# p768lwy3/torecsys

Hardware: AMD Instinct MI355X
Metric: CTR samples/sec fwd+bwd (DeepFM, 39 fields x dim 64) (higher is better)
Workload: dtype bf16; 1 GPU; BASELINE.json configs[1]: DeepFM 39 Criteo-shaped fields, MLP [400,400,400], 1000000 total rows, embed_dim 64, batch 65536, uniform indices, uniform field sizes; global_batch=65536, rows=1000000, parallelism=single, microbatches=1, optimizer=none, hipgraph=True, hipgraph_input_sets=1, hipgraph_steps_per_replay=4, fused_lookup_fm=True

## Files before the change

include/trs_abi.h:

```cpp
#ifndef TRS_ABI_H_
#define TRS_ABI_H_

#include <stddef.h>
#include <stdint.h>

#ifdef __cplusplus
extern "C" {
#endif

#define TRS_ABI_VERSION 3

enum { TRS_F32 = 0, TRS_BF16 = 1 };
enum { TRS_I64 = 0, TRS_I32 = 1 };
enum {
  TRS_OK = 0,
  TRS_EINVAL = -1,
  TRS_EDTYPE = -2,
  TRS_ESHAPE = -3,
  TRS_EALIGN = -4,
  TRS_ELAUNCH = -5,
  TRS_EWORKSPACE = -6
};

typedef void* trs_stream_t;
// ... 160 lines not shown
int trs_cin_bwd(const void* x0, const void* xk, const void* Wc, const void* gy, int64_t B, int32_t N,
                int32_t H, int32_t C, int32_t E, int32_t dtype, float* dWc, void* dx0, void* dxk,
                int32_t accumulate_dx0, trs_stream_t stream);

size_t trs_cin_cl_workspace_bytes(int32_t N, int32_t H, int32_t C);
int trs_cin_cl_fwd(const void* x0T, int32_t ld0, const void* xkT, int32_t ldk, const void* Wc,
                   const void* bias, int64_t B, int32_t N, int32_t H, int32_t C, int32_t E, int32_t dtype,
                   int32_t tri, void* yT, void* workspace, size_t ws_bytes, trs_stream_t stream);
size_t trs_cin_cl_bwd_data_workspace_bytes(int32_t N, int32_t H, int32_t C);
int trs_cin_cl_bwd_data(const void* x0T, int32_t ld0, const void* xkT, int32_t ldk, const void* gyT,
                        const void* Wc, int64_t B, int32_t N, int32_t H, int32_t C, int32_t E,
                        int32_t dtype, int32_t tri, void* dx0T, void* dxkT, int32_t ldo, void* workspace,
                        size_t ws_bytes, trs_stream_t stream);

size_t trs_cin_dw_workspace_bytes(int64_t B, int32_t N, int32_t H, int32_t C);
int trs_cin_dw(const void* gy, const void* x0, const void* xk, int64_t B, int32_t N, int32_t H, int32_t C,
               int32_t E, int32_t dtype, int32_t tri, float* dW, void* workspace, size_t ws_bytes,
               trs_stream_t stream);

int trs_cin_cl_bwd_data_live(const void* x0T, int32_t ld0, const void* xkT, int32_t ldk, const void* gyT, int32_t ldg,
                             const void* Wc, int64_t B, int32_t N, int32_t H, int32_t C, int32_t E, int32_t dtype,
                             void* dx0T, void* dxkT, int32_t ldo, void* workspace, size_t ws_bytes, trs_stream_t stream);
int trs_cin_dw_live(const void* gy, int64_t gy_batch_stride, const void* x0, const void* xk, int64_t B, int32_t N, int32_t H,
                    int32_t C, int32_t E, int32_t dtype, float* dW, void* workspace, size_t ws_bytes, trs_stream_t stream);

size_t trs_relu_bwd_bias_workspace_bytes(int64_t rows, int32_t C);
int trs_relu_bwd_bias(const void* gy, const void* y, int64_t rows, int32_t C, int32_t dtype, void* gz,
                      float* gb, void* workspace, size_t ws_bytes, trs_stream_t stream);

int trs_mlp_fused_supported(int32_t num_layers, const int32_t* widths);
#define TRS_MLP_FAMILY_AUTO 0
#define TRS_MLP_FAMILY_TILE 1
#define TRS_MLP_FAMILY_ROW_OWNER 2
#define TRS_MLP_FAMILY_MIXED 3
int32_t trs_mlp_fused_family(int32_t num_layers, const int32_t* widths, int64_t rows, int32_t request);
size_t trs_mlp_fused_workspace_bytes(int32_t num_layers, const int32_t* widths);
size_t trs_mlp_fused_mask_bytes(int64_t rows);
int trs_mlp_fused_fwd(const void* x, int64_t rows, int32_t num_layers, const int32_t* widths,
                      const void* const* weights, const void* const* biases, void* const* hidden, void* const* masks,
                      void* mask_in, void* y, int32_t dtype, int32_t family, int32_t x_stride, void* workspace,
                      size_t ws_bytes, trs_stream_t stream);
int trs_mlp_fused_bwd_data(const void* gy, int64_t rows, int32_t num_layers, const int32_t* widths,
                           const void* const* weights, const void* const* masks, void* const* gz, float* const* gbias,
                           void* gx, const void* mask_in, float* gbias_in, int32_t dtype, int32_t family,
                           void* workspace, size_t ws_bytes, trs_stream_t stream);
size_t trs_mlp_fused_bwd_wlast_part_bytes(int32_t num_layers, const int32_t* widths, int64_t rows, int32_t dtype,
                                          int32_t family, int32_t live);
int trs_mlp_fused_bwd_data_wlast(const void* gy, int32_t gy_stride, int64_t rows, int32_t num_layers,
                                 const int32_t* widths, const void* const* weights, const void* const* masks,
                                 void* const* gz, float* const* gbias, void* gx, const void* mask_in, float* gbias_in,
                                 const void* h_last, int32_t h_stride, int32_t live, float* wl_part,
                                 size_t wl_part_bytes, float* gw_last, int32_t dtype, int32_t family, void* workspace,
                                 size_t ws_bytes, trs_stream_t stream);

int trs_pad_cols(const void* src, int32_t c_in, void* dst, int32_t c_out, int64_t rows, int32_t dtype,
                 trs_stream_t stream);

size_t trs_rows_gemm_workspace_bytes(int32_t out_f, int32_t in_f);
int trs_rows_gemm_supported(int32_t out_f, int32_t in_f, int32_t x_stride);
int trs_rows_gemm(const void* x, int64_t rows, int32_t x_stride, const void* W, int32_t out_f, int32_t in_f,
                  int32_t dtype, void* y, void* workspace, size_t ws_bytes, trs_stream_t stream);

size_t trs_bucket_workspace_bytes(int64_t BN, int32_t world);
int trs_bucket_by_owner(const void* idx, int32_t idx_dtype, const int64_t* offsets, int64_t B, int32_t N,
                        int64_t rows_per_rank, int32_t world, int64_t* counts, int32_t* send_ids,
                        int32_t* send_pos, int32_t* inv_pos, void* workspace, size_t ws_bytes,
                        trs_stream_t stream);
int trs_embed_fm_sharded(const void* back, int64_t back_rows, const void* local, int64_t local_rows, int64_t n_valid,
                         int32_t E, int32_t dtype, const int32_t* inv_pos, const int32_t* send_ids, int32_t self_lo,
                         int32_t self_n, int64_t B, int32_t N, void* emb, void* fm, float* fm_sum, int32_t* err_flag,
                         trs_stream_t stream);
int trs_permute_grad(const void* g_block, const void* g_fm, const float* fm_sum, const void* x,
                     const int32_t* pos, int64_t K, int32_t N, int32_t E, int32_t dtype, void* out,
                     trs_stream_t stream);

int trs_bag_route_count(const void* idx, int32_t idx_dtype, int64_t B, int32_t L, int64_t V, int64_t rows_per_rank,
                        int32_t world, int32_t* counts, int32_t* err_flag, trs_stream_t stream);
int trs_bag_route_place(const void* idx, int32_t idx_dtype, int64_t B, int32_t L, int64_t V, int64_t rows_per_rank,
                        int32_t world, const int32_t* seg_start, int32_t* send_ids, int64_t n_send, trs_stream_t stream);
int trs_bag_pool_segments(const void* shard, int64_t n_valid, int32_t E, int32_t dtype, const int32_t* ids, int64_t n,
                          const int32_t* seg_start, int64_t S, float* out, int32_t* err_flag, trs_stream_t stream);
int trs_bag_combine(const float* parts, int32_t P, int64_t B, int32_t E, float scale, int32_t dtype, void* out,
                    trs_stream_t stream);
int trs_bag_expand_grad(const void* g_all, int32_t dtype, int32_t E, const int32_t* ids, int64_t n,
                        const int32_t* seg_start, int64_t S, int64_t n_valid, int64_t pad_local_row, void* grad_rows,
                        int32_t* ids_bwd, trs_stream_t stream);

int trs_rowdot_fwd(const void* h, const void* w, const void* bias, int64_t rows, int32_t C, int32_t dtype, void* out,
                   trs_stream_t stream);
size_t trs_rowdot_bwd_workspace_bytes(int64_t rows, int32_t C);
int trs_rowdot_bwd(const void* g, const void* h, const void* w, int64_t rows, int32_t C, int32_t dtype, void* gh,
                   float* gw, float* gb, void* workspace, size_t ws_bytes, trs_stream_t stream);

int trs_transpose_pad(const void* in, int64_t B, int32_t R, int32_t Cc, int32_t ld_in, void* out, int32_t ld_out,
                      int32_t dtype, trs_stream_t stream);

int trs_cat_head_fwd(const void* a, const void* d, const void* w, const void* bias, int64_t rows, int32_t N, int32_t Ea,
                     int32_t Eb, int32_t dtype, void* out, trs_stream_t stream);
size_t trs_cat_head_bwd_workspace_bytes(int64_t rows, int32_t N, int32_t Ea, int32_t Eb);
int trs_cat_head_bwd(const void* g, const void* a, const void* d, const void* w, int64_t rows, int32_t N, int32_t Ea,
                     int32_t Eb, int32_t dtype, void* ga, void* gd, float* gw, float* gb, void* workspace,
                     size_t ws_bytes, trs_stream_t stream);

int trs_wgrad_finish(const float* part, int32_t S, int32_t R, int32_t Cc, int32_t out_rows, int32_t out_cols,
                     int32_t dtype, void* gw, const float* gb_f32, void* gb, trs_stream_t stream);
int trs_wgrad_finish_t(const float* part, int32_t S, int32_t Cc, int32_t R, int32_t out_rows, int32_t out_cols,
                       int32_t dtype, void* gw, const float* gb_f32, void* gb, trs_stream_t stream);
int32_t trs_wgrad_rows_splits(int32_t M, int32_t N, int64_t rows);
int trs_wgrad_rows(const void* g, int32_t ldg, const void* x, int32_t ldx, int64_t rows, int32_t M, int32_t N,
                   int32_t dtype, int32_t S, float* part, trs_stream_t stream);
int32_t trs_wgrad_rows_many_splits(int32_t n_jobs, const int32_t* M, const int32_t* N, const int32_t* ldg,
                                   const int32_t* ldx, int64_t rows);
int32_t trs_wgrad_rows_many_map(int32_t n_jobs, const int32_t* M, const int32_t* N, const int32_t* ldg,
                                const int32_t* ldx, int64_t rows, int32_t block, int64_t* out);
int trs_wgrad_rows_many(int32_t n_jobs, const void* const* g, const int32_t* ldg, const void* const* x,
                        const int32_t* ldx, int64_t rows, const int32_t* M, const int32_t* N, int32_t S,
                        float* const* part, trs_stream_t stream);
int trs_wgrad_finish_many(int32_t n_jobs, const float* const* part, int32_t S, const int32_t* R, const int32_t* Cc,
                          const int32_t* out_rows, const int32_t* out_cols, int32_t dtype, void* const* gw,
                          const float* const* gb_f32, void* const* gb, trs_stream_t stream);
int32_t trs_wgrad_wide_splits(int32_t M_x, int32_t N_g, int32_t ld_g, int64_t rows);
int trs_wgrad_wide(const void* x, int32_t ldx, const void* g, int32_t ldg, int64_t rows, int32_t M_x, int32_t N_g,
                   int32_t S, float* part, trs_stream_t stream);
int32_t trs_wgrad_wide_many_splits(int32_t n_jobs, const int32_t* M_x, const int32_t* ldx, const int32_t* N_g,
                                   const int32_t* ldg, int64_t rows);
int32_t trs_wgrad_wide_many_map(int32_t n_jobs, const int32_t* M_x, const int32_t* ldx, const int32_t* N_g,
                                const int32_t* ldg, int64_t rows, int32_t block, int64_t* out);
int trs_wgrad_wide_many(int32_t n_jobs, const void* const* x, const int32_t* ldx, const void* const* g,
                        const int32_t* ldg, int64_t rows, const int32_t* M_x, const int32_t* N_g, int32_t S,
                        float* const* part, trs_stream_t stream);
int trs_wgrad_finish_t_many(int32_t n_jobs, const float* const* part, int32_t S, const int32_t* Cc, const int32_t* R,
                            const int32_t* out_rows, const int32_t* out_cols, int32_t dtype, void* const* gw,
                            const float* const* gb_f32, void* const* gb, trs_stream_t stream);
int trs_copy_padded_many(const int64_t* desc, int32_t n, int32_t elem_size, int64_t max_elems, trs_stream_t stream);

int32_t trs_cin_glue_blocks(int64_t B);
int trs_cin_glue_stats(const void* y, int64_t B, int32_t E, int32_t C, int32_t dtype, float* partial,
                       trs_stream_t stream);
int trs_cin_glue_fwd(const void* y, const float* scale, const float* shift, int64_t B, int32_t E, int32_t C, int32_t D,
                     int32_t Hs, int32_t dtype, void* hidden, void* pooled, trs_stream_t stream);
int trs_cin_glue_bwd_reduce(const void* y, const void* g_hidden, const void* g_pooled, const float* scale,
                            const float* shift, const float* mean, const float* invstd, int64_t B, int32_t E, int32_t C,
                            int32_t D, int32_t Hs, int32_t dtype, float* partial, trs_stream_t stream);
int trs_cin_glue_bwd_apply(const void* y, const void* g_hidden, const void* g_pooled, const float* scale,
                           const float* shift, const float* mean, const float* invstd, const float* c1, const float* c2,
                           int64_t B, int32_t E, int32_t C, int32_t D, int32_t Hs, int32_t dtype, void* gy,
                           trs_stream_t stream);
int trs_cin_glue_cf_supported(int32_t E, int32_t C);
int trs_cin_glue_fwd_cf(const void* y, const float* scale, const float* shift, int64_t B, int32_t E, int32_t C,
                        int32_t D, int32_t Hs, int32_t dtype, void* hidden, void* hidden_cf, void* pooled,
                        trs_stream_t stream);
int trs_cin_glue_bwd_apply_cf(const void* y, const void* g_hidden, const void* g_pooled, const float* scale,
                              const float* shift, const float* mean, const float* invstd, const float* c1,
                              const float* c2, int64_t B, int32_t E, int32_t C, int32_t D, int32_t Hs, int32_t dtype,
                              void* gy, void* gy_cf, float* colsum_partial, trs_stream_t stream);

int trs_opn_vec_fwd(const void* x, const void* kern, int32_t kern_is_num, int64_t B, int32_t N, int32_t E,
                    int32_t dtype, void* out, trs_stream_t stream);
size_t trs_opn_vec_bwd_workspace_bytes(int64_t B, int32_t N, int32_t E);
int trs_opn_vec_bwd(const void* g, const void* x, const void* kern, int32_t kern_is_num, int64_t B, int32_t N,
                    int32_t E, int32_t dtype, void* gx, float* gkern_vec, void* workspace, size_t ws_bytes,
                    trs_stream_t stream);

int trs_pair_mul_fwd(const void* a, const void* c, const void* bias, int32_t bias_per_pair, int64_t B, int32_t N,
                     int32_t E, int32_t dtype, void* out, trs_stream_t stream);
int trs_pair_mul_bwd(const void* g, const void* a, const void* c, int64_t B, int32_t N, int32_t E, int32_t dtype,
                     void* ga, void* gc, trs_stream_t stream);

int trs_rows_mul_bias_fwd(const void* a, const void* c, const void* bias, int32_t bias_per_pair, int64_t rows,
                          int32_t P, int32_t E, int32_t dtype, void* out, trs_stream_t stream);
int trs_rows_mul_bwd(const void* g, const void* a, const void* c, int64_t rows, int32_t E, int32_t dtype, void* ga,
                     void* gc, trs_stream_t stream);

int trs_pair_bilinear_fwd(const void* x, const void* W, int32_t w_per_pair, const void* bias, int32_t bias_per_pair,
                          int32_t mode, int64_t B, int32_t N, int32_t E, int32_t dtype, void* out,
                          trs_stream_t stream);
int trs_pair_bilinear_bwd_data(const void* g, const void* x, const void* W, int32_t w_per_pair, int32_t mode,
                               int64_t B, int32_t N, int32_t E, int32_t dtype, void* gx, void* gT,
                               trs_stream_t stream);

int trs_pair_bilinear_fwd_mfma(const void* x, const void* Wt, const void* bias, const int32_t* tasks, int32_t ntasks,
                               int32_t mode, int64_t B, int32_t N, int32_t E, int32_t dtype, void* out,
                               trs_stream_t stream);

int trs_pair_bilinear_bwd_data_mfma(const void* g, const void* x, const void* W, const void* Wt,
                                    const int32_t* tasks_i, int32_t nti, const int32_t* seg_i,
// ... 132 lines not shown
```

torecsys_amd/_abi.py:

```python
from __future__ import annotations

import ctypes
import os
import threading
from ctypes import c_char_p, c_int32, c_int64, c_size_t, c_void_p

import torch

_HERE = os.path.dirname(os.path.abspath(__file__))
LIB_PATH = os.environ.get("TRS_LIB_PATH") or os.path.join(_HERE, "libtrs_hip.so")

TRS_F32, TRS_BF16 = 0, 1
TRS_I64, TRS_I32 = 0, 1

_P, _I32, _I64, _SZ, _F32 = c_void_p, c_int32, c_int64, c_size_t, ctypes.c_float

_OPTIMIZER_TAIL = [_I32, _F32, _P, _F32, _F32, _F32, _P, _P, _P, _SZ, _P]

SIGNATURES = {
    "trs_version": (c_int32, []),
    "trs_last_error_string": (c_char_p, []),
    "trs_rowdot_fwd": (c_int32, [_P, _P, _P, _I64, _I32, _I32, _P, _P]),
    "trs_rowdot_bwd_workspace_bytes": (_SZ, [_I64, _I32]),
    "trs_rowdot_bwd": (c_int32, [_P, _P, _P, _I64, _I32, _I32, _P, _P, _P, _P, _SZ, _P]),
    "trs_transpose_pad": (c_int32, [_P, _I64, _I32, _I32, _I32, _P, _I32, _I32, _P]),
    "trs_cat_head_fwd": (c_int32, [_P, _P, _P, _P, _I64, _I32, _I32, _I32, _I32, _P, _P]),
    "trs_cat_head_bwd_workspace_bytes": (_SZ, [_I64, _I32, _I32, _I32]),
    "trs_cat_head_bwd": (c_int32, [_P, _P, _P, _P, _I64, _I32, _I32, _I32, _I32, _P, _P, _P, _P, _P, _SZ, _P]),
    "trs_wgrad_finish": (c_int32, [_P, _I32, _I32, _I32, _I32, _I32, _I32, _P, _P, _P, _P]),
    "trs_wgrad_finish_t": (c_int32, [_P, _I32, _I32, _I32, _I32, _I32, _I32, _P, _P, _P, _P]),
    "trs_wgrad_rows_splits": (c_int32, [_I32, _I32, _I64]),
    "trs_wgrad_rows": (c_int32, [_P, _I32, _P, _I32, _I64, _I32, _I32, _I32, _I32, _P, _P]),
    "trs_wgrad_rows_many_splits": (c_int32, [_I32, _P, _P, _P, _P, _I64]),
    "trs_wgrad_rows_many_map": (c_int32, [_I32, _P, _P, _P, _P, _I64, _I32, _P]),
    "trs_wgrad_rows_many": (c_int32, [_I32, _P, _P, _P, _P, _I64, _P, _P, _I32, _P, _P]),
    "trs_wgrad_finish_many": (c_int32, [_I32, _P, _I32, _P, _P, _P, _P, _I32, _P, _P, _P, _P]),
    "trs_wgrad_wide_splits": (c_int32, [_I32, _I32, _I32, _I64]),
    "trs_wgrad_wide": (c_int32, [_P, _I32, _P, _I32, _I64, _I32, _I32, _I32, _P, _P]),
    "trs_wgrad_wide_many_splits": (c_int32, [_I32, _P, _P, _P, _P, _I64]),
    "trs_wgrad_wide_many_map": (c_int32, [_I32, _P, _P, _P, _P, _I64, _I32, _P]),
    "trs_wgrad_wide_many": (c_int32, [_I32, _P, _P, _P, _P, _I64, _P, _P, _I32, _P, _P]),
    "trs_wgrad_finish_t_many": (c_int32, [_I32, _P, _I32, _P, _P, _P, _P, _I32, _P, _P, _P, _P]),
    "trs_copy_padded_many":(c_int32, [_P, _I32, _I32, _I64, _P]),
    "trs_cin_glue_blocks": (c_int32, [_I64]),
    "trs_cin_glue_stats": (c_int32, [_P, _I64, _I32, _I32, _I32, _P, _P]),
    "trs_cin_glue_fwd": (c_int32, [_P, _P, _P, _I64, _I32, _I32, _I32, _I32, _I32, _P, _P, _P]),
    "trs_cin_glue_bwd_reduce": (c_int32, [_P, _P, _P, _P, _P, _P, _P, _I64, _I32, _I32, _I32, _I32, _I32, _P, _P]),
    "trs_cin_glue_bwd_apply": (c_int32, [_P, _P, _P, _P, _P, _P, _P, _P, _P, _I64, _I32, _I32, _I32, _I32, _I32, _P, _P]),
    "trs_cin_glue_cf_supported": (c_int32, [_I32, _I32]),
    "trs_cin_glue_fwd_cf": (c_int32, [_P, _P, _P, _I64, _I32, _I32, _I32, _I32, _I32, _P, _P, _P, _P]),
    "trs_cin_glue_bwd_apply_cf": (c_int32, [_P, _P, _P, _P, _P, _P, _P, _P, _P, _I64, _I32, _I32, _I32, _I32, _I32, _P, _P, _P,
                                            _P]),
    "trs_opn_vec_fwd": (c_int32, [_P, _P, _I32, _I64, _I32, _I32, _I32, _P, _P]),
    "trs_opn_vec_bwd_workspace_bytes": (_SZ, [_I64, _I32, _I32]),
    "trs_opn_vec_bwd": (c_int32, [_P, _P, _P, _I32, _I64, _I32, _I32, _I32, _P, _P, _P, _SZ, _P]),
    "trs_pair_mul_fwd": (c_int32, [_P, _P, _P, _I32, _I64, _I32, _I32, _I32, _P, _P]),
    "trs_rows_mul_bias_fwd": (c_int32, [_P, _P, _P, _I32, _I64, _I32, _I32, _I32, _P, _P]),
    "trs_rows_mul_bwd": (c_int32, [_P, _P, _P, _I64, _I32, _I32, _P, _P, _P]),
    "trs_pair_mul_bwd": (c_int32, [_P, _P, _P, _I64, _I32, _I32, _I32, _P, _P, _P]),
    "trs_pair_bilinear_fwd": (c_int32, [_P, _P, _I32, _P, _I32, _I32, _I64, _I32, _I32, _I32, _P, _P]),
    "trs_pair_bilinear_bwd_data": (c_int32, [_P, _P, _P, _I32, _I32, _I64, _I32, _I32, _I32, _P, _P, _P]),
    "trs_pair_bilinear_fwd_mfma": (c_int32, [_P, _P, _P, _P, _I32, _I32, _I64, _I32, _I32, _I32, _P, _P]),
    "trs_pair_bilinear_bwd_data_mfma": (c_int32, [_P, _P, _P, _P, _P, _I32, _P, _P, _I32, _P, _I32, _I64, _I32, _I32, _I32,
                                                  _P, _P, _P, _P]),
    "trs_pair_bilinear_bwd_w_mfma_workspace_bytes": (_SZ, [_I64, _I32, _I32]),
    "trs_pair_bilinear_bwd_w_mfma": (c_int32, [_P, _P, _I32, _I64, _I32, _I32, _I32, _P, _P, _SZ, _P]),
    "trs_pair_epilogue_fwd": (c_int32, [_P, _P, _P, _I32, _I32, _I64, _I32, _I32, _I32, _P, _P]),
    "trs_pair_epilogue_bwd": (c_int32, [_P, _P, _P, _I32, _I64, _I32, _I32, _I32, _P, _P]),
    "trs_afm_fwd_dropout": (c_int32, [_P, _P, _P, _P, _P, _P, _F32, _I64, _I32, _I32, _I32, _I32, _P, _P, _P, _P]),
    "trs_afm_bwd_dropout": (c_int32, [_P, _P, _P, _P, _P, _F32, _P, _P, _P, _I64, _I32, _I32, _I32, _I32, _P, _P, _P, _P,
                                      _P, _P, _SZ, _P]),
    "trs_afm_pair_tiles": (c_int32, [_I32, _P, _I32, _P]),
    "trs_pad_cols": (c_int32, [_P, _I32, _P, _I32, _I64, _I32, _P]),
    "trs_rows_gemm_workspace_bytes": (_SZ, [_I32, _I32]),
    "trs_rows_gemm_supported": (c_int32, [_I32, _I32, _I32]),
    "trs_rows_gemm": (c_int32, [_P, _I64, _I32, _P, _I32, _I32, _I32, _P, _P, _SZ, _P]),
    "trs_afm_bwd_workspace_bytes": (_SZ, [_I64, _I32, _I32, _I32]),
    "trs_pack_columns": (c_int32, [_P, _P, _I32, _I32, _I64, _P, _I32, _P]),
    "trs_mark_timestamp": (c_int32, [_P, _I32, _P]),
    "trs_wall_clock_khz": (_I64, []),
    "trs_gather_rows": (c_int32, [_P, _I64, _I32, _I32, _P, _I32, _P, _I64, _I32, _P, _P, _P]),
    "trs_gather_rows_tables": (c_int32, [_P, _P, _I32, _I32, _P, _I32, _I64, _I32, _P, _P, _P]),
    "trs_fa_gather_rows": (c_int32, [_P, _I64, _I32, _I32, _P, _I32, _P, _I64, _I32, _P, _P, _P]),
    "trs_csr_workspace_bytes": (_SZ, [_I64, _I64]),
    "trs_csr_build": (c_int32, [_P, _I32, _P, _I64, _I32, _I64, _P, _P, _P, _SZ, _P, _P]),
    "trs_csr_build_skip": (c_int32, [_P, _I32, _P, _I64, _I32, _I64, _I64, _P, _P, _P, _SZ, _P, _P]),
    "trs_scatter_workspace_bytes": (_SZ, [_I64, _I32, _I32, _I32]),
    "trs_scatter_rows": (c_int32, [_P, _I64, _P, _I32, _P, _P, _P, _P, _I64, _I64, _I32, _I32, _I32, _I64, _P, _P, _SZ, _P]),
    "trs_scatter_rows_first": (c_int32, [_P, _I64, _P, _I32, _P, _P, _P, _P, _I64, _I64, _I32, _I32, _I32, _I64, _P, _P, _P, _P,
                                         _SZ, _P]),
    "trs_scatter_rows_update": (c_int32, [_P, _I64, _P, _I32, _P, _P, _P, _P, _I64, _I64, _I32, _I32, _I32, _I64,
                                          *_OPTIMIZER_TAIL]),
    "trs_scatter_rows_update_mapped": (c_int32, [_P, _P, _P, _P, _P, _I64, _I64, _I64, _I32, _I32, *_OPTIMIZER_TAIL]),
    "trs_adam_step_size": (c_int32, [_P, _P, ctypes.c_double, ctypes.c_double, _P, _P]),
    "trs_compact_rows_slots": (_I64, [_I64]),
# ... 43 lines not shown
    "trs_senet_bwd_workspace_bytes": (_SZ, [_I64, _I32, _I32]),
    "trs_senet_bwd": (c_int32, [_P, _P, _P, _P, _P, _P, _I64, _I32, _I32, _I32, _I32, _P, _P, _P, _P, _P, _P, _SZ, _P]),
    "trs_senet_squeeze": (c_int32, [_P, _I64, _I32, _I32, _I32, _P, _P]),
    "trs_senet_scale_fwd": (c_int32, [_P, _P, _I64, _I32, _I32, _I32, _P, _P]),
    "trs_senet_scale_bwd": (c_int32, [_P, _P, _P, _P, _I64, _I32, _I32, _I32, _P, _P, _P]),
    "trs_moe_gate_vector_shape": (c_int32, [_I32, _I32]),
    "trs_moe_gate_last_path": (c_int32, []),
    "trs_moe_gate_fwd": (c_int32, [_P, _P, _P, _I64, _I32, _I32, _I32, _P, _P]),
    "trs_moe_gate_bwd": (c_int32, [_P, _P, _P, _P, _I64, _I32, _I32, _I32, _P, _P, _P]),
    "trs_dynamic_routing_path": (c_int32, [_I32, _I32, _I32, _I32]),
    "trs_dynamic_routing_fwd": (c_int32, [_P, _P, _I64, _I32, _I32, _I32, _I32, _I32, _P, _P, _P, _P]),
    "trs_dynamic_routing_bwd": (c_int32, [_P, _P, _P, _P, _I64, _I32, _I32, _I32, _I32, _P, _P]),
    "trs_seq_rnn_path": (c_int32, [_I32, _I32, _I32, _I32]),
    "trs_seq_rnn_workspace_bytes": (_SZ, [_I32, _I32]),
    "trs_seq_rnn_fwd": (c_int32, [_P, _I64, _I32, _I32, _P, _I32, _P, _I32, _I64, _I32, _P, _P, _P, _P, _I32, _I32, _I32, _P,
                                  _P, _P, _P, _P, _SZ, _P, _P]),
    "trs_seq_rnn_bwd": (c_int32, [_P, _I64, _I32, _I32, _P, _I32, _P, _I32, _I64, _I32, _P, _P, _P, _P, _I32, _I32, _P, _P,
                                  _P, _P, _P, _P, _P, _SZ, _P]),
    "trs_fm_fwd": (c_int32, [_P, _I64, _I32, _I32, _I32, _P, _P, _P]),
    "trs_fm_bwd": (c_int32, [_P, _P, _P, _I64, _I32, _I32, _I32, _P, _P]),
    "trs_pair_dot_fwd": (c_int32, [_P, _I64, _I32, _I32, _I32, _P, _P]),
    "trs_embed_pair_dot": (c_int32, [_P, _I64, _I32, _I32, _P, _I32, _P, _I64, _I32, _P, _P, _P, _P]),
    "trs_pair_dot_bwd": (c_int32, [_P, _P, _I64, _I32, _I32, _I32, _P, _P]),
    "trs_ffm_fwd": (c_int32, [_P, _I64, _I32, _I32, _I32, _P, _P]),
    "trs_ffm_bwd": (c_int32, [_P, _P, _I64, _I32, _I32, _I32, _P, _P]),
    "trs_ffm_fused_fwd": (c_int32, [_P, _I64, _I32, _I32, _P, _I32, _P, _I64, _I32, _P, _P, _P]),
    "trs_ffm_fused_bwd": (c_int32, [_P, _I64, _I32, _I32, _P, _I32, _P, _P, _P, _P, _I64, _I32, _P, _P, _P]),
    "trs_cross_workspace_bytes": (_SZ, [_I64, _I32, _I32, _I32]),
    "trs_cross_fwd": (c_int32, [_P, _P, _P, _I64, _I32, _I32, _I32, _P, _P, _SZ, _P]),
    "trs_cross_bwd": (c_int32, [_P, _P, _P, _P, _I64, _I32, _I32, _I32, _I32, _P, _P, _P, _P, _SZ, _P]),
    "trs_cin_fwd": (c_int32, [_P, _P, _P, _P, _I64, _I32, _I32, _I32, _I32, _I32, _P, _P, _P]),
    "trs_cin_bwd": (c_int32, [_P, _P, _P, _P, _I64, _I32, _I32, _I32, _I32, _I32, _P, _P, _P, _I32, _P]),
    "trs_cin_cl_workspace_bytes": (_SZ, [_I32, _I32, _I32]),
    "trs_cin_cl_fwd": (c_int32, [_P, _I32, _P, _I32, _P, _P, _I64, _I32, _I32, _I32, _I32, _I32, _I32, _P, _P, _SZ, _P]),
    "trs_cin_cl_bwd_data_workspace_bytes": (_SZ, [_I32, _I32, _I32]),
    "trs_cin_cl_bwd_data": (c_int32, [_P, _I32, _P, _I32, _P, _P, _I64, _I32, _I32, _I32, _I32, _I32, _I32, _P, _P, _I32,
                                      _P, _SZ, _P]),
    "trs_cin_dw_workspace_bytes": (_SZ, [_I64, _I32, _I32, _I32]),
    "trs_cin_dw": (c_int32, [_P, _P, _P, _I64, _I32, _I32, _I32, _I32, _I32, _I32, _P, _P, _SZ, _P]),
    "trs_cin_cl_bwd_data_live": (c_int32, [_P, _I32, _P, _I32, _P, _I32, _P, _I64, _I32, _I32, _I32, _I32, _I32, _P, _P, _I32,
                                           _P, _SZ, _P]),
    "trs_cin_dw_live": (c_int32, [_P, _I64, _P, _P, _I64, _I32, _I32, _I32, _I32, _I32, _P, _P, _SZ, _P]),
    "trs_relu_bwd_bias_workspace_bytes": (_SZ, [_I64, _I32]),
    "trs_relu_bwd_bias": (c_int32, [_P, _P, _I64, _I32, _I32, _P, _P, _P, _SZ, _P]),
    "trs_mlp_fused_supported": (c_int32, [_I32, _P]),
    "trs_mlp_fused_family": (c_int32, [_I32, _P, _I64, _I32]),
    "trs_mlp_fused_workspace_bytes": (_SZ, [_I32, _P]),
    "trs_mlp_fused_mask_bytes": (_SZ, [_I64]),
    "trs_mlp_fused_fwd": (c_int32, [_P, _I64, _I32, _P, _P, _P, _P, _P, _P, _P, _I32, _I32, _I32, _P, _SZ, _P]),
    "trs_mlp_fused_bwd_data": (c_int32, [_P, _I64, _I32, _P, _P, _P, _P, _P, _P, _P, _P, _I32, _I32, _P, _SZ, _P]),
    "trs_mlp_fused_bwd_wlast_part_bytes": (_SZ, [_I32, _P, _I64, _I32, _I32, _I32]),
    "trs_mlp_fused_bwd_data_wlast": (c_int32, [_P, _I32, _I64, _I32, _P, _P, _P, _P, _P, _P, _P, _P, _P, _I32, _I32, _P, _SZ, _P,
                                               _I32, _I32, _P, _SZ, _P]),
    "trs_ctr_logit_fwd": (c_int32, [_P, _I32, _P, _I32, _P, _P, _I32, _P, _I64, _I32, _P, _P]),
    "trs_bce_logits_workspace_bytes": (_SZ, [_I64]),
    "trs_bce_logits_fwd": (c_int32, [_P, _I32, _P, _I32, _I64, _P, _P, _SZ, _P]),
    "trs_bce_logits_bwd": (c_int32, [_P, _I32, _P, _I32, _P, _I64, _P, _P]),
    "trs_pair_score_path": (c_int32, [_I32, _I32]),
    "trs_embed_pair_score_fwd": (c_int32, [_P, _I64, _P, _I64, _P, _I64, _P, _I64, _I32, _I32, _I32, _I64, _I32, _I32, _P,
                                           _I32, _P, _P]),
    "trs_pair_score_bwd_workspace_bytes": (_SZ, [_I64, _I32, _I32, _I32]),
    "trs_embed_pair_score_bwd": (c_int32, [_P, _I64, _P, _I64, _P, _I64, _P, _I64, _I32, _I32, _I32, _I64, _I32, _I32, _P,
                                           _I32, _P, _P, _SZ, _P]),
    "trs_rank_loss_workspace_bytes": (_SZ, [_I64]),
    "trs_rank_loss_fwd": (c_int32, [_P, _I64, _P, _I64, _I32, _P, _I64, _I32, _I32, _F32, _I32, _P, _P, _P, _SZ, _P]),
    "trs_rank_loss_bwd": (c_int32, [_P, _I64, _P, _I64, _I32, _P, _I64, _I32, _I32, _F32, _I32, _P, _P, _P, _I64, _P, _I64,
                                    _P]),
    "trs_bucket_workspace_bytes": (_SZ, [_I64, _I32]),
    "trs_bucket_by_owner": (c_int32, [_P, _I32, _P, _I64, _I32, _I64, _I32, _P, _P, _P, _P, _P, _SZ, _P]),
    "trs_embed_fm_sharded": (c_int32, [_P, _I64, _P, _I64, _I64, _I32, _I32, _P, _P, _I32, _I32, _I64, _I32, _P, _P, _P, _P,
                                       _P]),
    "trs_permute_grad": (c_int32, [_P, _P, _P, _P, _P, _I64, _I32, _I32, _I32, _P, _P]),
    "trs_bag_route_count": (c_int32, [_P, _I32, _I64, _I32, _I64, _I64, _I32, _P, _P, _P]),
    "trs_bag_route_place": (c_int32, [_P, _I32, _I64, _I32, _I64, _I64, _I32, _P, _P, _I64, _P]),
    "trs_bag_pool_segments": (c_int32, [_P, _I64, _I32, _I32, _P, _I64, _P, _I64, _P, _P, _P]),
    "trs_bag_combine": (c_int32, [_P, _I32, _I64, _I32, _F32, _I32, _P, _P]),
    "trs_bag_expand_grad": (c_int32, [_P, _I32, _I32, _P, _I64, _P, _I64, _I64, _I64, _P, _P, _P]),
}

_lib = None
_lock = threading.Lock()


def load() -> ctypes.CDLL:
    global _lib
    if _lib is not None:
        return _lib
    with _lock:
        if _lib is not None:
            return _lib
        if not os.path.exists(LIB_PATH):
            raise RuntimeError(
                f"torecsys_amd: HIP library not built ({LIB_PATH} missing). Run "
                "`python -m torecsys_amd.build` (or __graft_entry__.build()). There is no CPU fallback.")
        lib = ctypes.CDLL(LIB_PATH)
        for name, (res, args) in SIGNATURES.items():
            try:
                fn = getattr(lib, name)
            except AttributeError as e:
                raise RuntimeError(f"torecsys_amd: {LIB_PATH} does not export {name}; rebuild it") from e
            fn.restype = res
            fn.argtypes = args
        _lib = lib
    return _lib


# ... 52 lines not shown
            _HipEvent._free.append(self.h)
            self.h = None


_MARK_CAP = 4096
_rings = {}


def _mark_ring(name: str) -> torch.Tensor:
    r = _rings.get(name)
    if r is None:
        raise RuntimeError(f"time_kernel({name!r}) must be enabled before the capture starts")
    return r


_every = {}


def time_kernel(name: str, enable: bool = True, expect: int = 0, every: int = 1):
    if enable:
        _timed[name] = []
        _every[name] = [max(1, int(every)), 0]
        _rings[name] = torch.zeros(_MARK_CAP + 1, dtype=torch.int64, device="cuda")
        fresh = [_HipEvent() for _ in range(max(0, 2 * expect - len(_HipEvent._free)))]
        for ev in fresh:
            ev.release()
    else:
        _timed.pop(name, None)
        _rings.pop(name, None)
        _every.pop(name, None)


def kernel_times_ms(name: str):
    torch.cuda.synchronize()
    ev = _timed.get(name, [])
    out = [a.elapsed_time(b) for a, b in ev]
    for a, b in ev:
        a.release()
        b.release()
    ev.clear()
    ring = _rings.get(name)
    if ring is not None:
        host = ring.cpu()
        n = int(host[0])
        if n > _MARK_CAP:
            n = 0
        khz = float(load().trs_wall_clock_khz())
        if khz > 0:
            out += [float(host[2 + 2 * j] - host[1 + 2 * j]) / khz for j in range(n // 2)]
        ring.zero_()
    return out


def call(name: str, *args):
    rec = _timed.get(name)
    if rec is not None:
        st = stream_ptr()
        if torch.cuda.is_current_stream_capturing():
            ring = _mark_ring(name)
            lib = load()
            lib.trs_mark_timestamp(ctypes.c_void_p(ring.data_ptr()), _MARK_CAP, st)
            rc = getattr(lib, name)(*args)
            lib.trs_mark_timestamp(ctypes.c_void_p(ring.data_ptr()), _MARK_CAP, st)
        else:
            ev = _every[name]
            ev[1] += 1
            if ev[1] % ev[0] == 0:
                a, b = _HipEvent(), _HipEvent()
                a.record(st, 0)
                rc = getattr(load(), name)(*args)
                b.record(st, 0)
                rec.append((a, b))
            else:
                rc = getattr(load(), name)(*args)
    else:
        rc = getattr(load(), name)(*args)
    if rc != 0:
        raise RuntimeError(f"{name} failed (code {rc}): {last_error()}")


def size_query(name: str, *args) -> int:
    return int(getattr(load(), name)(*args))


def value_dtype_code(t: torch.Tensor) -> int:
    if t.dtype == torch.float32:
        return TRS_F32
    if t.dtype == torch.bfloat16:
        return TRS_BF16
    raise TypeError(f"torecsys_amd: unsupported value dtype {t.dtype} (float32 and bfloat16 only)")


def index_dtype_code(t: torch.Tensor) -> int:
    if t.dtype == torch.int64:
        return TRS_I64
    if t.dtype == torch.int32:
        return TRS_I32
    raise TypeError(f"torecsys_amd: unsupported index dtype {t.dtype}")


def current_stream_of(dev: torch.device) -> torch.cuda.Stream:
    return torch.cuda.current_stream(dev.index if dev.index is not None else torch._C._cuda_getDevice())


def require_device(*tensors: torch.Tensor) -> torch.device:
    dev = None
    for t in tensors:
        if t is None:
            continue
        if not t.is_cuda:
            raise RuntimeError(
                "torecsys_amd: tensors must be on a HIP ('cuda') device; this package has no CPU path "
                f"(got a tensor on {t.device})")
        if dev is None:
            dev = t.device
        elif t.device != dev:
            raise RuntimeError(f"torecsys_amd: tensors on different devices ({dev} vs {t.device})")
    if dev is not None and dev.index is not None and dev.index != torch._C._cuda_getDevice():
# ... 13 lines not shown
```

torecsys_amd/csrc/mlp_epilogue.hip:

```cpp
#include <algorithm>

#include "trs_common.hpp"

namespace trs {

constexpr int RB_THREADS = 256;

template <typename T>
__global__ __launch_bounds__(RB_THREADS) void relu_bwd_bias_kernel(const uint4* __restrict__ gy, const uint4* __restrict__ y,
                                                                   uint4* __restrict__ gz, float* __restrict__ part,
                                                                   int64_t rows, int vpr ,
                                                                   int rows_per_band) {
  constexpr int VE = Vec16<T>::VE;
  __shared__ float red[RB_THREADS][VE];
  const int64_t r0 = (int64_t)blockIdx.x * rows_per_band;
  const int64_t r1 = r0 + rows_per_band < rows ? r0 + rows_per_band : rows;
  const int cv = threadIdx.x % vpr, rl = threadIdx.x / vpr, rstep = RB_THREADS / vpr;
  float acc[VE];
#pragma unroll
  for (int k = 0; k < VE; ++k) acc[k] = 0.f;
  if (rl < rstep) {
    constexpr int U = 4;
    for (int64_t rb = r0 + rl; rb < r1; rb += (int64_t)rstep * U) {
      uint4 gv[U], yv[U];
// ... 158 lines not shown
        if (v == 0) gb += gr[u];
      }
      if (gh != nullptr) {
        float o[VE];
#pragma unroll
        for (int k = 0; k < VE; ++k) o[k] = gr[u] * wv[k];
        gh[r * lpr + v] = Vec16<T>::pack(o);
      }
    }
  }
  if (partial == nullptr) return;
#pragma unroll
  for (int k = 0; k < VE; ++k) red[threadIdx.x][k] = gw[k];
  red[threadIdx.x][VE] = gb;
  __syncthreads();
  if (rr == 0) {
    float* mine = partial + (size_t)blockIdx.x * (C + 1);
#pragma unroll
    for (int k = 0; k < VE; ++k) {
      float t = 0.f;
      for (int q = 0; q < rpp; ++q) t += red[q * lpr + v][k];
      mine[v * VE + k] = t;
    }
    if (v == 0) {
      float t = 0.f;
      for (int q = 0; q < rpp; ++q) t += red[q * lpr][VE];
      mine[C] = t;
    }
  }
}

__global__ void rowdot_finish_kernel(const float* __restrict__ tmp, int C, float* __restrict__ gw,
                                         float* __restrict__ gb) {
  const int c = blockIdx.x * blockDim.x + threadIdx.x;
  if (c < C) gw[c] = tmp[c];
  else if (c == C) gb[0] = tmp[C];
}

static int rowdot_fwd_blocks(int64_t rows, int lpr) {
  const int rpp = 256 / lpr;
  return (int)std::min<int64_t>((rows + (int64_t)rpp * 4 - 1) / ((int64_t)rpp * 4), 8192);
}
static int rowdot_blocks(int64_t rows, int lpr) {
  const int rpp = 256 / lpr;
  return (int)std::min<int64_t>((rows + rpp - 1) / rpp, 1023);
}
static bool rowdot_shape_ok(int C, int dtype) {
  const int ve = dtype == TRS_F32 ? 4 : 8;
  const int lpr = C % ve == 0 ? C / ve : 0;
  return lpr >= 1 && lpr <= 64 && (lpr & (lpr - 1)) == 0;
}

template <typename T>
__device__ __forceinline__ void wgrad_finish_body(const float* __restrict__ part, int S, int R, int Cc, int out_rows,
                                                  int out_cols, T* __restrict__ gw, const float* __restrict__ gbf,
                                                  T* __restrict__ gb) {
  const int c = blockIdx.x * 256 + threadIdx.x;
  if ((int)blockIdx.y == out_rows) {
    if (gb != nullptr && c < out_rows) gb[c] = from_f32<T>(gbf[c]);
    return;
  }
  if ((int)blockIdx.y > out_rows || c >= out_cols) return;
  const int r = blockIdx.y;
  const float* p = part + (size_t)r * Cc + c;
  const size_t stride = (size_t)R * Cc;
  float a0 = 0.f, a1 = 0.f, a2 = 0.f, a3 = 0.f;
  int s = 0;
  for (; s + 4 <= S; s += 4) {
    a0 += p[(size_t)s * stride];
    a1 += p[(size_t)(s + 1) * stride];
    a2 += p[(size_t)(s + 2) * stride];
    a3 += p[(size_t)(s + 3) * stride];
  }
  for (; s < S; ++s) a0 += p[(size_t)s * stride];
  gw[(size_t)r * out_cols + c] = from_f32<T>((a0 + a1) + (a2 + a3));
}

template <typename T>
__global__ __launch_bounds__(256) void wgrad_finish_kernel(const float* __restrict__ part, int S, int R, int Cc,
                                                          int out_rows, int out_cols, T* __restrict__ gw,
                                                          const float* __restrict__ gbf, T* __restrict__ gb) {
  wgrad_finish_body<T>(part, S, R, Cc, out_rows, out_cols, gw, gbf, gb);
}

constexpr int WF_MAXJ = 8;
struct WgradFinishJob {
  const float* part;
  void* gw;
  const float* gbf;
  void* gb;
  int R, Cc, out_rows, out_cols;
};
struct WgradFinishArgs {
  WgradFinishJob job[WF_MAXJ];
  int S;
};
template <typename T>
__global__ __launch_bounds__(256) void wgrad_finish_many_kernel(WgradFinishArgs a) {
  const WgradFinishJob& j = a.job[blockIdx.z];
  if (j.part == nullptr) {
    const int c = blockIdx.x * 256 + threadIdx.x;
    if (blockIdx.y == 0 && c < j.out_cols) ((T*)j.gb)[c] = from_f32<T>(j.gbf[c]);
    return;
  }
  wgrad_finish_body<T>(j.part, a.S, j.R, j.Cc, j.out_rows, j.out_cols, (T*)j.gw, j.gbf, (T*)j.gb);
}

constexpr int WF_SL = 16;
constexpr int WF_COLS = 256 / WF_SL;
template <typename T>
__global__ __launch_bounds__(256) void wgrad_finish_few_rows_kernel(const float* __restrict__ part, int S, int R, int Cc,
                                                                   int out_rows, int out_cols, T* __restrict__ gw,
                                                                   const float* __restrict__ gbf, T* __restrict__ gb) {
  __shared__ float red[WF_SL][WF_COLS + 1];
  if ((int)blockIdx.y == out_rows) {
    const int c = blockIdx.x * 256 + threadIdx.x;
    if (gb != nullptr && c < out_rows) gb[c] = from_f32<T>(gbf[c]);
    return;
  }
  const int cl = threadIdx.x % WF_COLS, sl = threadIdx.x / WF_COLS;
  const int c = blockIdx.x * WF_COLS + cl;
  const int r = blockIdx.y;
  const size_t stride = (size_t)R * Cc;
  float a0 = 0.f, a1 = 0.f, a2 = 0.f, a3 = 0.f;
  if (c < out_cols) {
    const float* p = part + (size_t)r * Cc + c;
    int s = sl;
    for (; s + 3 * WF_SL < S; s += 4 * WF_SL) {
      a0 += p[(size_t)s * stride];
      a1 += p[(size_t)(s + WF_SL) * stride];
      a2 += p[(size_t)(s + 2 * WF_SL) * stride];
      a3 += p[(size_t)(s + 3 * WF_SL) * stride];
    }
    for (; s < S; s += WF_SL) a0 += p[(size_t)s * stride];
  }
  red[sl][cl] = (a0 + a1) + (a2 + a3);
  __syncthreads();
  if (sl == 0 && c < out_cols) {
    float t = 0.f;
#pragma unroll
    for (int k = 0; k < WF_SL; ++k) t += red[k][cl];
    gw[(size_t)r * out_cols + c] = from_f32<T>(t);
  }
}

template <typename T>
__device__ __forceinline__ void wgrad_finish_t_body(const float* __restrict__ part, int S, int Cc, int R, int out_rows,
                                                    int out_cols, T* __restrict__ gw, const float* __restrict__ gbf,
                                                    T* __restrict__ gb) {
  __shared__ float tile[32][33];
  const int tx = threadIdx.x & 31, ty = threadIdx.x >> 5;
  if ((int)blockIdx.y == (out_cols + 31) / 32) {
    const int r = blockIdx.x * 32 + tx;
    if (gb != nullptr && ty == 0 && r < out_rows) gb[r] = from_f32<T>(gbf[r]);
    return;
  }
  const int r0 = blockIdx.x * 32, c0 = blockIdx.y * 32;
  const size_t stride = (size_t)Cc * R;
  float acc[4] = {0.f, 0.f, 0.f, 0.f};
#pragma unroll
  for (int i = 0; i < 4; ++i) {
    const int c = c0 + ty + 8 * i, r = r0 + tx;
    if (c < out_cols && r < out_rows) {
      const float* p = part + (size_t)c * R + r;
      float a0 = 0.f, a1 = 0.f;
      int sidx = 0;
      for (; sidx + 2 <= S; sidx += 2) {
        a0 += p[(size_t)sidx * stride];
        a1 += p[(size_t)(sidx + 1) * stride];
      }
      if (sidx < S) a0 += p[(size_t)sidx * stride];
      acc[i] = a0 + a1;
    }
  }
#pragma unroll
  for (int i = 0; i < 4; ++i) tile[ty + 8 * i][tx] = acc[i];
  __syncthreads();
#pragma unroll
  for (int i = 0; i < 4; ++i) {
    const int r = r0 + ty + 8 * i, c = c0 + tx;
    if (r < out_rows && c < out_cols) gw[(size_t)r * out_cols + c] = from_f32<T>(tile[tx][ty + 8 * i]);
  }
}

template <typename T>
__global__ __launch_bounds__(256) void wgrad_finish_t_kernel(const float* __restrict__ part, int S, int Cc, int R,
                                                            int out_rows, int out_cols, T* __restrict__ gw,
                                                            const float* __restrict__ gbf, T* __restrict__ gb) {
  wgrad_finish_t_body<T>(part, S, Cc, R, out_rows, out_cols, gw, gbf, gb);
}

template <typename T>
__global__ __launch_bounds__(256) void wgrad_finish_t_many_kernel(WgradFinishArgs a) {
  const WgradFinishJob& j = a.job[blockIdx.z];
  if (j.part == nullptr) {
    const int c = (blockIdx.y * gridDim.x + blockIdx.x) * 256 + threadIdx.x;
    if (c < j.out_cols) ((T*)j.gb)[c] = from_f32<T>(j.gbf[c]);
    return;
  }
  if ((int)blockIdx.x >= (j.out_rows + 31) / 32 || (int)blockIdx.y > (j.out_cols + 31) / 32) return;
  wgrad_finish_t_body<T>(j.part, a.S, j.Cc, j.R, j.out_rows, j.out_cols, (T*)j.gw, j.gbf, (T*)j.gb);
}

}

using namespace trs;

extern "C" int trs_rowdot_fwd(const void* h, const void* w, const void* bias, int64_t rows, int32_t C, int32_t dtype,
                              void* out, trs_stream_t stream) {
  TRS_REQUIRE(rows >= 0 && C > 0, TRS_EINVAL, "rowdot_fwd: bad size");
  if (rows == 0) return TRS_OK;
  TRS_REQUIRE(h && w && out, TRS_EINVAL, "rowdot_fwd: NULL pointer");
  TRS_REQUIRE(dtype == TRS_F32 || dtype == TRS_BF16, TRS_EDTYPE, "rowdot_fwd: dtype %d", dtype);
  TRS_REQUIRE(rowdot_shape_ok(C, dtype), TRS_ESHAPE, "rowdot_fwd: C = %d (C*elem/16 must be a power of two <= 64)", C);
  TRS_REQUIRE(aligned16(h) && aligned16(w), TRS_EALIGN, "rowdot_fwd: 16-byte alignment");
  const int lpr = C / (dtype == TRS_F32 ? 4 : 8);
  hipStream_t s = (hipStream_t)stream;
  if (dtype == TRS_F32)
    hipLaunchKernelGGL((rowdot_fwd_kernel<float>), dim3(rowdot_fwd_blocks(rows, lpr)), dim3(256), 0, s, (const uint4*)h,
                       (const uint4*)w, (const float*)bias, rows, lpr, (float*)out);
  else
    hipLaunchKernelGGL((rowdot_fwd_kernel<bf16_t>), dim3(rowdot_fwd_blocks(rows, lpr)), dim3(256), 0, s, (const uint4*)h,
                       (const uint4*)w, (const bf16_t*)bias, rows, lpr, (bf16_t*)out);
  return check_launch("rowdot_fwd");
}

extern "C" size_t trs_rowdot_bwd_workspace_bytes(int64_t rows, int32_t C) {
  return (size_t)1024 * (size_t)(C + 1) * 4 + 256;
}

extern "C" int trs_rowdot_bwd(const void* g, const void* h, const void* w, int64_t rows, int32_t C, int32_t dtype,
                              void* gh, float* gw, float* gb, void* workspace, size_t ws_bytes, trs_stream_t stream) {
  TRS_REQUIRE(rows >= 0 && C > 0, TRS_EINVAL, "rowdot_bwd: bad size");
  if (rows == 0) return TRS_OK;
  TRS_REQUIRE(g && h && w, TRS_EINVAL, "rowdot_bwd: NULL pointer");
  TRS_REQUIRE((gw == nullptr) == (gb == nullptr), TRS_EINVAL, "rowdot_bwd: gw and gb go together");
  TRS_REQUIRE(dtype == TRS_F32 || dtype == TRS_BF16, TRS_EDTYPE, "rowdot_bwd: dtype %d", dtype);
  TRS_REQUIRE(rowdot_shape_ok(C, dtype), TRS_ESHAPE, "rowdot_bwd: C = %d (C*elem/16 must be a power of two <= 64)", C);
  TRS_REQUIRE(aligned16(h) && aligned16(w) && aligned16(gh), TRS_EALIGN, "rowdot_bwd: 16-byte alignment");
  TRS_REQUIRE(gw == nullptr || (workspace != nullptr && ws_bytes >= trs_rowdot_bwd_workspace_bytes(rows, C)),
              TRS_EWORKSPACE, "rowdot_bwd: workspace too small");
  const int lpr = C / (dtype == TRS_F32 ? 4 : 8);
  const int grid = rowdot_blocks(rows, lpr);
  hipStream_t s = (hipStream_t)stream;
  float* part = gw != nullptr ? (float*)workspace : nullptr;
  if (dtype == TRS_F32)
    hipLaunchKernelGGL((rowdot_bwd_kernel<float>), dim3(grid), dim3(256), 0, s, (const float*)g, (const uint4*)h,
                       (const uint4*)w, rows, lpr, (uint4*)gh, part);
  else
    hipLaunchKernelGGL((rowdot_bwd_kernel<bf16_t>), dim3(grid), dim3(256), 0, s, (const bf16_t*)g, (const uint4*)h,
                       (const uint4*)w, rows, lpr, (uint4*)gh, part);
  if (gw != nullptr) {
    float* tmp = part + (size_t)grid * (C + 1);
    if (grid >= 1024) return fail(TRS_EWORKSPACE, "rowdot_bwd: internal workspace layout");
// ... 245 lines not shown
  TRS_REQUIRE(row_bytes % 16 == 0 && row_bytes / 16 <= RB_THREADS, TRS_ESHAPE,
              "relu_bwd_bias: row bytes %d must be a multiple of 16 and at most %d", row_bytes, RB_THREADS * 16);
  if (rows == 0) {
    return zero_bytes(gb, (size_t)C * 4, s);
  }
  TRS_REQUIRE(gy && y && gz, TRS_EINVAL, "relu_bwd_bias: NULL pointer");
  TRS_REQUIRE(aligned16(gy) && aligned16(y) && aligned16(gz), TRS_EALIGN, "relu_bwd_bias: 16-byte alignment");
  const int vpr = row_bytes / 16;
  int nbands = (int)std::min<int64_t>(1024, (rows + 31) / 32);
  const int rows_per_band = (int)((rows + nbands - 1) / nbands);
  nbands = (int)((rows + rows_per_band - 1) / rows_per_band);
  TRS_REQUIRE(ws_bytes >= (size_t)nbands * C * 4, TRS_EWORKSPACE, "relu_bwd_bias: workspace too small");
  float* part = (float*)workspace;
  if (dtype == TRS_F32)
    hipLaunchKernelGGL((relu_bwd_bias_kernel<float>), dim3(nbands), dim3(RB_THREADS), 0, s, (const uint4*)gy,
                       (const uint4*)y, (uint4*)gz, part, rows, vpr, rows_per_band);
  else
    hipLaunchKernelGGL((relu_bwd_bias_kernel<bf16_t>), dim3(nbands), dim3(RB_THREADS), 0, s, (const uint4*)gy,
                       (const uint4*)y, (uint4*)gz, part, rows, vpr, rows_per_band);
  hipLaunchKernelGGL(colsum_partials_kernel, dim3((C + 15) / 16), dim3(256), 0, s, part, nbands, C, gb);
  return check_launch("relu_bwd_bias");
}

extern "C" int trs_wgrad_finish(const float* part, int32_t S, int32_t R, int32_t Cc, int32_t out_rows, int32_t out_cols,
                                int32_t dtype, void* gw, const float* gb_f32, void* gb, trs_stream_t stream) {
  TRS_REQUIRE(S > 0 && R > 0 && Cc > 0 && out_rows > 0 && out_cols > 0 && out_rows <= R && out_cols <= Cc, TRS_EINVAL,
              "wgrad_finish: bad size");
  TRS_REQUIRE(part && gw, TRS_EINVAL, "wgrad_finish: NULL pointer");
  TRS_REQUIRE((gb == nullptr) == (gb_f32 == nullptr), TRS_EINVAL, "wgrad_finish: gb and gb_f32 go together");
  TRS_REQUIRE(dtype == TRS_F32 || dtype == TRS_BF16, TRS_EDTYPE, "wgrad_finish: dtype %d", dtype);
  TRS_REQUIRE(gb == nullptr || out_rows <= ((out_cols + 255) / 256) * 256, TRS_ESHAPE,
              "wgrad_finish: out_rows %d exceeds the bias row of workgroups", out_rows);
  hipStream_t s = (hipStream_t)stream;
  dim3 grid((out_cols + 255) / 256, out_rows + 1);
  if (S >= 4 * WF_SL && (int64_t)grid.x * out_rows < 64) {
    dim3 gridf((out_cols + WF_COLS - 1) / WF_COLS, out_rows + 1);
    if (dtype == TRS_F32)
      hipLaunchKernelGGL((wgrad_finish_few_rows_kernel<float>), gridf, dim3(256), 0, s, part, S, R, Cc, out_rows, out_cols,
                         (float*)gw, gb_f32, (float*)gb);
    else
      hipLaunchKernelGGL((wgrad_finish_few_rows_kernel<bf16_t>), gridf, dim3(256), 0, s, part, S, R, Cc, out_rows, out_cols,
                         (bf16_t*)gw, gb_f32, (bf16_t*)gb);
    return check_launch("wgrad_finish");
  }
  if (dtype == TRS_F32)
    hipLaunchKernelGGL((wgrad_finish_kernel<float>), grid, dim3(256), 0, s, part, S, R, Cc, out_rows, out_cols,
                       (float*)gw, gb_f32, (float*)gb);
  else
    hipLaunchKernelGGL((wgrad_finish_kernel<bf16_t>), grid, dim3(256), 0, s, part, S, R, Cc, out_rows, out_cols,
                       (bf16_t*)gw, gb_f32, (bf16_t*)gb);
  return check_launch("wgrad_finish");
}

extern "C" int trs_wgrad_finish_many(int32_t n_jobs, const float* const* part, int32_t S, const int32_t* R,
                                     const int32_t* Cc, const int32_t* out_rows, const int32_t* out_cols, int32_t dtype,
                                     void* const* gw, const float* const* gb_f32, void* const* gb, trs_stream_t stream) {
  TRS_REQUIRE(n_jobs >= 1 && n_jobs <= WF_MAXJ, TRS_EINVAL, "wgrad_finish_many: %d jobs (1 .. %d)", n_jobs, WF_MAXJ);
  TRS_REQUIRE(part && R && Cc && out_rows && out_cols && gw && gb_f32 && gb, TRS_EINVAL, "wgrad_finish_many: NULL array");
  TRS_REQUIRE(S > 0, TRS_EINVAL, "wgrad_finish_many: bad size");
  TRS_REQUIRE(dtype == TRS_F32 || dtype == TRS_BF16, TRS_EDTYPE, "wgrad_finish_many: dtype %d", dtype);
  WgradFinishArgs a{};
  a.S = S;
  int max_rows = 0, max_cols = 0;
  for (int k = 0; k < n_jobs; ++k) {
    if (part[k] == nullptr) {
      TRS_REQUIRE(gw[k] == nullptr && gb[k] && gb_f32[k] && out_cols[k] > 0, TRS_EINVAL,
                  "wgrad_finish_many: a job without a product takes gb_f32, gb and out_cols only (job %d)", k);
      a.job[k] = WgradFinishJob{nullptr, nullptr, gb_f32[k], gb[k], 0, 0, 0, out_cols[k]};
      max_cols = std::max(max_cols, out_cols[k]);
      continue;
    }
    TRS_REQUIRE(R[k] > 0 && Cc[k] > 0 && out_rows[k] > 0 && out_cols[k] > 0 && out_rows[k] <= R[k] && out_cols[k] <= Cc[k],
                TRS_EINVAL, "wgrad_finish_many: bad size (job %d)", k);
    TRS_REQUIRE(part[k] && gw[k], TRS_EINVAL, "wgrad_finish_many: NULL pointer (job %d)", k);
    TRS_REQUIRE((gb[k] == nullptr) == (gb_f32[k] == nullptr), TRS_EINVAL, "wgrad_finish_many: gb and gb_f32 go together (job %d)", k);
    TRS_REQUIRE(gb[k] == nullptr || out_rows[k] <= ((out_cols[k] + 255) / 256) * 256, TRS_ESHAPE,
                "wgrad_finish_many: out_rows %d exceeds the bias row of workgroups", out_rows[k]);
    a.job[k] = WgradFinishJob{part[k], gw[k], gb_f32[k], gb[k], R[k], Cc[k], out_rows[k], out_cols[k]};
    max_rows = std::max(max_rows, out_rows[k]);
    max_cols = std::max(max_cols, out_cols[k]);
  }
  dim3 grid((max_cols + 255) / 256, max_rows + 1, n_jobs);
  if (dtype == TRS_F32)
    hipLaunchKernelGGL((wgrad_finish_many_kernel<float>), grid, dim3(256), 0, (hipStream_t)stream, a);
  else
    hipLaunchKernelGGL((wgrad_finish_many_kernel<bf16_t>), grid, dim3(256), 0, (hipStream_t)stream, a);
  return check_launch("wgrad_finish_many");
}

extern "C" int trs_wgrad_finish_t(const float* part, int32_t S, int32_t Cc, int32_t R, int32_t out_rows, int32_t out_cols,
                                  int32_t dtype, void* gw, const float* gb_f32, void* gb, trs_stream_t stream) {
  TRS_REQUIRE(S > 0 && R > 0 && Cc > 0 && out_rows > 0 && out_cols > 0 && out_rows <= R && out_cols <= Cc, TRS_EINVAL,
              "wgrad_finish_t: bad size");
  TRS_REQUIRE(part && gw, TRS_EINVAL, "wgrad_finish_t: NULL pointer");
  TRS_REQUIRE((gb == nullptr) == (gb_f32 == nullptr), TRS_EINVAL, "wgrad_finish_t: gb and gb_f32 go together");
  TRS_REQUIRE(dtype == TRS_F32 || dtype == TRS_BF16, TRS_EDTYPE, "wgrad_finish_t: dtype %d", dtype);
  hipStream_t s = (hipStream_t)stream;
  dim3 grid((out_rows + 31) / 32, (out_cols + 31) / 32 + 1);
  if (dtype == TRS_F32)
    hipLaunchKernelGGL((wgrad_finish_t_kernel<float>), grid, dim3(256), 0, s, part, S, Cc, R, out_rows, out_cols,
                       (float*)gw, gb_f32, (float*)gb);
  else
    hipLaunchKernelGGL((wgrad_finish_t_kernel<bf16_t>), grid, dim3(256), 0, s, part, S, Cc, R, out_rows, out_cols,
                       (bf16_t*)gw, gb_f32, (bf16_t*)gb);
  return check_launch("wgrad_finish_t");
}

extern "C" int trs_wgrad_finish_t_many(int32_t n_jobs, const float* const* part, int32_t S, const int32_t* Cc,
                                       const int32_t* R, const int32_t* out_rows, const int32_t* out_cols, int32_t dtype,
                                       void* const* gw, const float* const* gb_f32, void* const* gb, trs_stream_t stream) {
  TRS_REQUIRE(n_jobs >= 1 && n_jobs <= WF_MAXJ, TRS_EINVAL, "wgrad_finish_t_many: %d jobs (1 .. %d)", n_jobs, WF_MAXJ);
  TRS_REQUIRE(part && R && Cc && out_rows && out_cols && gw && gb_f32 && gb, TRS_EINVAL, "wgrad_finish_t_many: NULL array");
  TRS_REQUIRE(S > 0, TRS_EINVAL, "wgrad_finish_t_many: bad size");
  TRS_REQUIRE(dtype == TRS_F32 || dtype == TRS_BF16, TRS_EDTYPE, "wgrad_finish_t_many: dtype %d", dtype);
  WgradFinishArgs a{};
  a.S = S;
  int gx = 1, gy = 1;
  for (int k = 0; k < n_jobs; ++k) {
    if (part[k] == nullptr) {
      TRS_REQUIRE(gw[k] == nullptr && gb[k] && gb_f32[k] && out_cols[k] > 0, TRS_EINVAL,
                  "wgrad_finish_t_many: a job without a product takes gb_f32, gb and out_cols only (job %d)", k);
      a.job[k] = WgradFinishJob{nullptr, nullptr, gb_f32[k], gb[k], 0, 0, 0, out_cols[k]};
      continue;
    }
    TRS_REQUIRE(R[k] > 0 && Cc[k] > 0 && out_rows[k] > 0 && out_cols[k] > 0 && out_rows[k] <= R[k] && out_cols[k] <= Cc[k],
                TRS_EINVAL, "wgrad_finish_t_many: bad size (job %d)", k);
    TRS_REQUIRE(part[k] && gw[k], TRS_EINVAL, "wgrad_finish_t_many: NULL pointer (job %d)", k);
    TRS_REQUIRE((gb[k] == nullptr) == (gb_f32[k] == nullptr), TRS_EINVAL, "wgrad_finish_t_many: gb and gb_f32 go together (job %d)", k);
    a.job[k] = WgradFinishJob{part[k], gw[k], gb_f32[k], gb[k], R[k], Cc[k], out_rows[k], out_cols[k]};
    gx = std::max(gx, (out_rows[k] + 31) / 32);
    gy = std::max(gy, (out_cols[k] + 31) / 32 + 1);
  }
  for (int k = 0; k < n_jobs; ++k)
    if (part[k] == nullptr && (out_cols[k] + 255) / 256 > gx * gy) gx = ((out_cols[k] + 255) / 256 + gy - 1) / gy;
  dim3 grid(gx, gy, n_jobs);
  if (dtype == TRS_F32)
    hipLaunchKernelGGL((wgrad_finish_t_many_kernel<float>), grid, dim3(256), 0, (hipStream_t)stream, a);
  else
    hipLaunchKernelGGL((wgrad_finish_t_many_kernel<bf16_t>), grid, dim3(256), 0, (hipStream_t)stream, a);
  return check_launch("wgrad_finish_t_many");
}

namespace trs {
__global__ __launch_bounds__(256) void copy_padded_many_kernel(const int64_t* __restrict__ desc, int elem_size) {
  const int64_t* d = desc + (size_t)blockIdx.y * 6;
  const char* src = reinterpret_cast<const char*>(d[0]);
  char* dst = reinterpret_cast<char*>(d[1]);
  const int64_t rows = d[2], cols = d[3], sld = d[4], dld = d[5];
  const int64_t rb = cols * elem_size;
  const bool vec = rb % 16 == 0 && (sld * elem_size) % 16 == 0 && (dld * elem_size) % 16 == 0 &&
                   (d[0] & 15) == 0 && (d[1] & 15) == 0;
  const int64_t stride = (int64_t)gridDim.x * blockDim.x;
  if (vec) {
    const int64_t vpr = rb / 16, total = rows * vpr;
    for (int64_t t = (int64_t)blockIdx.x * blockDim.x + threadIdx.x; t < total; t += stride) {
      const int64_t r = t / vpr, c = t - r * vpr;
      *reinterpret_cast<uint4*>(dst + r * dld * elem_size + c * 16) =
          *reinterpret_cast<const uint4*>(src + r * sld * elem_size + c * 16);
    }
  } else {
    const int64_t total = rows * rb;
    for (int64_t t = (int64_t)blockIdx.x * blockDim.x + threadIdx.x; t < total; t += stride) {
      const int64_t r = t / rb, c = t - r * rb;
      dst[r * dld * elem_size + c] = src[r * sld * elem_size + c];
    }
  }
}
}

namespace trs {
__global__ __launch_bounds__(256) void pad_cols_kernel(const uint16_t* __restrict__ src, int c_in, uint16_t* __restrict__ dst,
                                                       int c_out, int64_t total) {
  const int64_t stride = (int64_t)gridDim.x * blockDim.x;
  for (int64_t t = (int64_t)blockIdx.x * blockDim.x + threadIdx.x; t < total; t += stride) {
    const int64_t r = t / c_out;
    const int c = (int)(t - r * c_out);
    dst[t] = c < c_in ? src[r * c_in + c] : (uint16_t)0;
  }
}
}

extern "C" int trs_pad_cols(const void* src, int32_t c_in, void* dst, int32_t c_out, int64_t rows, int32_t dtype,
                            trs_stream_t stream) {
  TRS_REQUIRE(dtype == TRS_BF16, TRS_EDTYPE, "pad_cols: bf16 only");
  TRS_REQUIRE(c_in > 0 && c_out >= c_in && rows >= 0, TRS_ESHAPE, "pad_cols: %d -> %d columns", c_in, c_out);
  if (rows == 0) return TRS_OK;
  TRS_REQUIRE(src && dst, TRS_EINVAL, "pad_cols: NULL pointer");
  const int64_t total = rows * c_out;
  hipLaunchKernelGGL(trs::pad_cols_kernel, dim3(trs::stream_grid(total, 256, 2048)), dim3(256), 0, (hipStream_t)stream,
                     (const uint16_t*)src, c_in, (uint16_t*)dst, c_out, total);
  return trs::check_launch("pad_cols");
}

// ... 11 lines not shown
```

torecsys_amd/csrc/mlp_fused.hip:

```cpp
#include <algorithm>

#include "trs_common.hpp"

namespace trs {

typedef __attribute__((ext_vector_type(8))) __bf16 mf_bf16x8;
typedef __attribute__((ext_vector_type(4))) float mf_f32x4;
typedef __attribute__((ext_vector_type(4))) unsigned mf_u32x4;

constexpr int MF_ROWS = 128;
constexpr int MF_MT = MF_ROWS / 16;
constexpr int MF_WAVES = 8;
constexpr int MF_MINW = 2;
constexpr int MF_MAXP = 2;
constexpr int MF_MAXL = 8;
constexpr int MF_MAXLIVE = 3;
constexpr int MF_MASK_TILE = 64 * MF_WAVES * 16;

__host__ __device__ __forceinline__ int mf_col_of_slot(int mt, int m) {
  return 32 * (mt >> 1) + 8 * (m >> 2) + 4 * (mt & 1) + (m & 3);
}

__global__ __launch_bounds__(256) void mlp_prepack_kernel(const bf16_t* __restrict__ W, const bf16_t* __restrict__ b,
                                                          int out_f, int in_f, int transpose, int NTt ,
// ... 870 lines not shown
  MlpArgs a;
  a.nsteps = L;
  a.in = x;
  a.in_stride = widths[0];
  a.rows = rows;
  a.nbias = 0;
  a.act_str = mlp_act_str(L, widths);
  a.mask_in = (uint8_t*)mask_in;
  a.colsum_in = nullptr;
  char* wsp = (char*)workspace;
  float* bias_base = (float*)(wsp + mlp_frag_bytes(L, widths));
  size_t woff = 0, boff = 0;
  MlpPackArgs pk;
  const int pk_blocks = mlp_fwd_pack_jobs(L, widths, weights, biases, wsp, pk.job);
  for (int l = 0; l < L; ++l) {
    const int K = pad32(widths[l]), N = pad32(widths[l + 1]);
    bf16_t* wf = (bf16_t*)(wsp + woff);
    float* bf = bias_base + boff;
    MlpStep& st = a.step[l];
    st.wf = (const uint4*)wf;
    st.bias = bf;
    st.K = K;
    st.N = N;
    st.relu = l + 1 < L ? 1 : 0;
    st.out = l + 1 < L ? hidden[l] : y;
    st.out_stride = l + 1 < L ? N : widths[L];
    st.mask = l + 1 < L ? (uint8_t*)masks[l] : nullptr;
    st.colsum = nullptr;
    woff += (size_t)K * N * 2;
    boff += N;
  }
  hipLaunchKernelGGL(mlp_prepack_many_kernel, dim3(pk_blocks, L), dim3(256), 0, s, pk);
  a.nbias = (int)boff;
  const size_t lds = (size_t)MF_ROWS * a.act_str + boff * 4;
  static bool attr = false;
  if (!attr) {
    if (hipFuncSetAttribute((const void*)mlp_fused_fwd_kernel, hipFuncAttributeMaxDynamicSharedMemorySize, 160 * 1024) !=
        hipSuccess)
      return check_launch("mlp_fused_fwd: LDS attribute");
    attr = true;
  }
  const int64_t ntiles = (rows + MF_ROWS - 1) / MF_ROWS;
  hipLaunchKernelGGL(mlp_fused_fwd_kernel, dim3((int)std::min<int64_t>(ntiles, MF_GRID)), dim3(64 * MF_WAVES), lds, s, a);
  return check_launch("mlp_fused_fwd");
}

namespace trs {
struct MlpWlast {
  const void* h_last;
  int h_stride, live, gy_stride;
  float* part;
  float* gw;
};
static size_t mlp_bwd_lds(int L, const int32_t* widths, int live) {
  return (size_t)MF_ROWS * mlp_act_str(L, widths) + 8 * 512 * 4 + (size_t)(L + 1 + live) * 512 * 4;
}
static int mlp_bwd_grid(int64_t rows) { return (int)std::min<int64_t>((rows + MF_ROWS - 1) / MF_ROWS, MF_GRID); }
}

static int mlp_fused_bwd_impl(const void* gy, int64_t rows, int32_t num_layers, const int32_t* widths,
                              const void* const* weights, const void* const* masks, void* const* gz,
                              float* const* gbias, void* gx, const void* mask_in, float* gbias_in, int32_t dtype,
                              int32_t family, void* workspace, size_t ws_bytes, trs_stream_t stream, const MlpWlast* wl) {
  hipStream_t s = (hipStream_t)stream;
  TRS_REQUIRE(dtype == TRS_BF16, TRS_EDTYPE, "mlp_fused_bwd_data: bf16 only");
  TRS_REQUIRE(trs_mlp_fused_supported(num_layers, widths), TRS_ESHAPE, "mlp_fused_bwd_data: unsupported layer widths");
  TRS_REQUIRE(weights && workspace && gy && masks && gz && gbias, TRS_EINVAL, "mlp_fused_bwd_data: NULL pointer");
  TRS_REQUIRE(ws_bytes >= trs_mlp_fused_workspace_bytes(num_layers, widths), TRS_EWORKSPACE,
              "mlp_fused_bwd_data: workspace too small");
  const int L = num_layers;
  bool fam_ok = (family == TRS_MLP_FAMILY_TILE || family == TRS_MLP_FAMILY_ROW_OWNER || family == TRS_MLP_FAMILY_MIXED) &&
                mlp_resolve_family(L, widths, rows, family) == family;
  if (!fam_ok && family == TRS_MLP_FAMILY_MIXED && L <= MF_MAXL) {
    int32_t wn[MF_MAXL + 1];
    for (int l = 0; l <= L; ++l) wn[l] = widths[l];
    for (int w0 = pad32(widths[0]) - 32; w0 >= 32 && !fam_ok; w0 -= 32) {
      wn[0] = w0;
      fam_ok = mlp_resolve_family(L, wn, rows, family) == family;
    }
  }
  TRS_REQUIRE(fam_ok, TRS_EINVAL,
              "mlp_fused_bwd_data: family must be the TILE / ROW_OWNER / MIXED value the forward ran under (got %d)", family);
  TRS_REQUIRE(family != TRS_MLP_FAMILY_ROW_OWNER || gx != nullptr, TRS_EINVAL, "mlp_fused_bwd_data: the row-owner kernels need gx");
  TRS_REQUIRE((mask_in == nullptr) == (gbias_in == nullptr) && (mask_in == nullptr || (L + 1 <= MF_MAXL && gx != nullptr)),
              TRS_EINVAL, "mlp_fused_bwd_data: mask_in and gbias_in come together (and with gx, at most %d layers)", MF_MAXL - 1);
  if (rows == 0) {
    for (int l = 0; l < L; ++l)
      if (int rc = zero_bytes(gbias[l], (size_t)pad32(widths[l + 1]) * 4, s)) return rc;
    if (wl)
      if (int rc = zero_bytes(wl->gw, (size_t)wl->live * pad32(widths[L - 1]) * 4, s)) return rc;
    if (gbias_in) return zero_bytes(gbias_in, (size_t)pad32(widths[0]) * 4, s);
    return TRS_OK;
  }
  if (family == TRS_MLP_FAMILY_ROW_OWNER) {
    RoColsum rc;
    const int rcode = mlp_ro_bwd(gy, rows, L, widths, weights, masks, gz, gbias, gx, mask_in, gbias_in, workspace, s, &rc);
    if (rcode != TRS_OK) return rcode;
    MlpColsumArgs cs;
    cs.nparts = rc.nparts;
    int kmax = 0;
    for (int i = 0; i < rc.count; ++i) {
      cs.part[i] = rc.part[i];
      cs.out[i] = rc.out[i];
      cs.n[i] = cs.stride[i] = rc.n[i];
      kmax = std::max(kmax, rc.n[i]);
    }
    hipLaunchKernelGGL(mlp_colsum_reduce_many_kernel, dim3((kmax + 63) / 64, rc.count), dim3(1024), 0, s, cs);
    return check_launch("mlp_fused_bwd_data");
  }
  MlpArgs a;
  a.nsteps = L;
  a.in = gy;
  a.in_stride = widths[L];
  a.rows = rows;
  a.nbias = 0;
  a.act_str = mlp_act_str(L, widths);
  const int grid = mlp_bwd_grid(rows);
  a.h_last = wl ? wl->h_last : nullptr;
  a.h_stride = wl ? wl->h_stride : 0;
  a.live = wl ? wl->live : 0;
  a.wl_part = wl ? wl->part : nullptr;
  a.in_narrow = wl && wl->gy_stride != widths[L] ? wl->gy_stride : 0;
  char* wsp = (char*)workspace;
  float* part_base = (float*)(wsp + mlp_frag_bytes(L, widths));
  size_t woff = 0, poff = 0;
  MlpPackArgs pk;
  const int pk_blocks = mlp_bwd_pack_jobs(L, widths, weights, wsp, pk.job);
  for (int sidx = 0; sidx < L; ++sidx) {
    const int l = L - 1 - sidx;
    const int K = pad32(widths[l + 1]), N = pad32(widths[l]);
    bf16_t* wf = (bf16_t*)(wsp + woff);
    MlpStep& st = a.step[sidx];
    st.wf = (const uint4*)wf;
    st.bias = nullptr;
    st.K = K;
    st.N = N;
    st.relu = 0;
    st.out = l > 0 ? gz[l - 1] : gx;
    st.out_stride = l > 0 ? N : widths[0];
    st.mask = l > 0 ? (uint8_t*)masks[l - 1] : (uint8_t*)mask_in;
    st.colsum = part_base + poff;
    woff += (size_t)K * N * 2;
    poff += (size_t)grid * K;
  }
  a.mask_in = nullptr;
  a.colsum_in = mask_in != nullptr ? part_base + poff : nullptr;
  a.ro_masks = family == TRS_MLP_FAMILY_MIXED ? 1 : 0;
  const size_t lds = mlp_bwd_lds(L, widths, a.live);
  static bool attr = false;
  if (!attr) {
    for (const void* k : {(const void*)mlp_fused_bwd_kernel<false>, (const void*)mlp_fused_bwd_kernel<true>,
                          (const void*)mlp_fused_bwd_wlast_kernel<false>, (const void*)mlp_fused_bwd_wlast_kernel<true>})
      if (hipFuncSetAttribute(k, hipFuncAttributeMaxDynamicSharedMemorySize, 160 * 1024) != hipSuccess)
        return check_launch("mlp_fused_bwd_data: LDS attribute");
    attr = true;
  }
  hipLaunchKernelGGL(mlp_prepack_many_kernel, dim3(pk_blocks, L), dim3(256), 0, s, pk);
  auto* kern = a.ro_masks ? (wl ? mlp_fused_bwd_wlast_kernel<true> : mlp_fused_bwd_kernel<true>)
                          : (wl ? mlp_fused_bwd_wlast_kernel<false> : mlp_fused_bwd_kernel<false>);
  hipLaunchKernelGGL(kern, dim3(grid), dim3(64 * MF_WAVES), lds, s, a);
  MlpColsumArgs cs;
  cs.nparts = grid;
  int kmax = 0;
  for (int sidx = 0; sidx < L; ++sidx) {
    const int l = L - 1 - sidx;
    cs.part[sidx] = a.step[sidx].colsum;
    cs.out[sidx] = gbias[l];
    cs.n[sidx] = cs.stride[sidx] = a.step[sidx].K;
    kmax = std::max(kmax, a.step[sidx].K);
  }
  int nsum = L;
  if (a.colsum_in != nullptr) {
    cs.part[L] = a.colsum_in;
    cs.out[L] = gbias_in;
    cs.n[L] = cs.stride[L] = pad32(widths[0]);
    kmax = std::max(kmax, cs.n[L]);
    nsum = L + 1;
  }
  for (int j = 0; j < a.live; ++j, ++nsum) {
    const int Kh = pad32(widths[L - 1]);
    cs.part[nsum] = wl->part + (size_t)j * Kh;
    cs.out[nsum] = wl->gw + (size_t)j * Kh;
    cs.n[nsum] = Kh;
    cs.stride[nsum] = a.live * Kh;
    kmax = std::max(kmax, Kh);
  }
  hipLaunchKernelGGL(mlp_colsum_reduce_many_kernel, dim3((kmax + 63) / 64, nsum), dim3(1024), 0, s, cs);
  return check_launch("mlp_fused_bwd_data");
}

extern "C" int trs_mlp_fused_bwd_data(const void* gy, int64_t rows, int32_t num_layers, const int32_t* widths,
                                      const void* const* weights, const void* const* masks, void* const* gz,
                                      float* const* gbias, void* gx, const void* mask_in, float* gbias_in, int32_t dtype,
                                      int32_t family, void* workspace, size_t ws_bytes, trs_stream_t stream) {
  return mlp_fused_bwd_impl(gy, rows, num_layers, widths, weights, masks, gz, gbias, gx, mask_in, gbias_in, dtype, family,
                            workspace, ws_bytes, stream, nullptr);
}

extern "C" size_t trs_mlp_fused_bwd_wlast_part_bytes(int32_t num_layers, const int32_t* widths, int64_t rows, int32_t dtype,
                                                     int32_t family, int32_t live) {
  const int L = num_layers;
  if (dtype != TRS_BF16 || rows <= 0 || L < 2 || !mlp_fused_covers(L, widths)) return 0;
  if (family != TRS_MLP_FAMILY_TILE && family != TRS_MLP_FAMILY_MIXED) return 0;
  if (live < 1 || live > MF_MAXLIVE || live > widths[L]) return 0;
  if (L + 1 + live > MF_MAXL) return 0;
  if (mlp_bwd_lds(L, widths, live) > 160 * 1024) return 0;
  return (size_t)mlp_bwd_grid(rows) * live * pad32(widths[L - 1]) * 4;
}

extern "C" int trs_mlp_fused_bwd_data_wlast(const void* gy, int32_t gy_stride, int64_t rows, int32_t num_layers,
                                            const int32_t* widths, const void* const* weights, const void* const* masks,
                                            void* const* gz, float* const* gbias, void* gx, const void* mask_in,
                                            float* gbias_in, const void* h_last, int32_t h_stride, int32_t live,
// ... 16 lines not shown
              "mlp_fused_bwd_data_wlast: 16-byte alignment");
  const MlpWlast wl{h_last, h_stride, live, gy_stride, wl_part, gw_last};
  return mlp_fused_bwd_impl(gy, rows, num_layers, widths, weights, masks, gz, gbias, gx, mask_in, gbias_in, dtype, family,
                            workspace, ws_bytes, stream, &wl);
}

extern "C" size_t trs_rows_gemm_workspace_bytes(int32_t out_f, int32_t in_f) {
  if (out_f <= 0 || in_f <= 0) return 256;
  return (size_t)pad32(out_f) * pad32(in_f) * 2 + 256;
}

extern "C" int trs_rows_gemm_supported(int32_t out_f, int32_t in_f, int32_t x_stride) {
  if (out_f < 8 || out_f > 512 || in_f < 32 || in_f % 8 != 0 || x_stride % 8 != 0 || x_stride < pad32(out_f)) return 0;
  const size_t lds = (size_t)MF_ROWS * (pad32(out_f) * 2 + 16);
  return lds <= 160 * 1024 ? 1 : 0;
}

extern "C" int trs_rows_gemm(const void* x, int64_t rows, int32_t x_stride, const void* W, int32_t out_f, int32_t in_f,
                             int32_t dtype, void* y, void* workspace, size_t ws_bytes, trs_stream_t stream) {
  hipStream_t s = (hipStream_t)stream;
  TRS_REQUIRE(dtype == TRS_BF16, TRS_EDTYPE, "rows_gemm: bf16 only");
  TRS_REQUIRE(trs_rows_gemm_supported(out_f, in_f, x_stride), TRS_ESHAPE, "rows_gemm: unsupported shape (K %d, N %d)", out_f, in_f);
  TRS_REQUIRE(W && workspace && x && y, TRS_EINVAL, "rows_gemm: NULL pointer");
  TRS_REQUIRE(ws_bytes >= trs_rows_gemm_workspace_bytes(out_f, in_f), TRS_EWORKSPACE, "rows_gemm: workspace too small");
  TRS_REQUIRE(aligned16(x) && aligned16(y) && aligned16(workspace), TRS_EALIGN, "rows_gemm: 16-byte alignment");
  if (rows == 0) return TRS_OK;
  const int K = pad32(out_f), N = pad32(in_f);
  MlpPackArgs pk;
  const int pk_blocks = mlp_gemm_pack_job(W, out_f, in_f, workspace, pk.job);
  hipLaunchKernelGGL(mlp_prepack_many_kernel, dim3(pk_blocks, 1), dim3(256), 0, s, pk);
  RowsGemmArgs a;
  a.in = x;
  a.wf = (const uint4*)workspace;
  a.out = y;
  a.rows = rows;
  a.in_stride = x_stride;
  a.K = K;
  a.N = N;
  a.out_cols = in_f;
  a.out_stride = in_f;
  a.act_str = K * 2 + 16;
  const size_t lds = (size_t)MF_ROWS * a.act_str;
  static bool attr = false;
  if (!attr) {
    if (hipFuncSetAttribute((const void*)mlp_rows_gemm_kernel, hipFuncAttributeMaxDynamicSharedMemorySize, 160 * 1024) !=
        hipSuccess)
      return check_launch("rows_gemm: LDS attribute");
    attr = true;
  }
  const int64_t ntiles = (rows + MF_ROWS - 1) / MF_ROWS;
  hipLaunchKernelGGL(mlp_rows_gemm_kernel, dim3((int)std::min<int64_t>(ntiles, MF_GRID)), dim3(64 * MF_WAVES), lds, s, a);
  return check_launch("rows_gemm");
}
```

torecsys_amd/csrc/scatter.hip:

```cpp
#include <algorithm>

#include "trs_common.hpp"

namespace trs {

constexpr int SCAN_THREADS = 256;
constexpr int SCAN_ITEMS = 16;
constexpr int SCAN_TILE = SCAN_THREADS * SCAN_ITEMS;
constexpr int LONG_ROW = 64;
constexpr int LONG_ROW_ELEM = 32;
constexpr int LONG_CHUNK = 256;
constexpr int ELEM_SPLIT = 2048;

template <typename IdxT, bool SKIP = false>
__global__ __launch_bounds__(256) void csr_count_kernel(const IdxT* __restrict__ idx,
                                                        const int64_t* __restrict__ offsets, int64_t BN, int N,
                                                        int64_t V, int32_t* __restrict__ count,
                                                        int32_t* __restrict__ slot, int32_t* __restrict__ err_flag,
                                                        const int32_t* __restrict__ gate, int64_t skip_row = -1) {
  constexpr int U = 4;
  if (gate != nullptr && *gate == 0) return;
  const unsigned n_items = (unsigned)BN, uN = (unsigned)N;
  const unsigned stride = gridDim.x * blockDim.x;
  for (unsigned p0 = blockIdx.x * blockDim.x + threadIdx.x; p0 < n_items; p0 += stride * U) {
// ... 771 lines not shown
__global__ __launch_bounds__(256) void scatter_long_rows_finish_kernel(
    const float* __restrict__ fm_sum, const uint4* __restrict__ table, const int32_t* __restrict__ row_start,
    uint4* __restrict__ grad, const int32_t* __restrict__ long_rows, const float* __restrict__ scratch, RowSink sink) {
  constexpr int L = 1 << LOG2L;
  constexpr int VE = Vec16<T>::VE;
  const int lane_v = threadIdx.x & (L - 1);
  const int nlong = long_rows[0];
  const int groups = (gridDim.x * blockDim.x) >> LOG2L;
  for (int i = (blockIdx.x * blockDim.x + threadIdx.x) >> LOG2L; i < nlong; i += groups) {
    if (long_rows[2 + 2 * i] != 0) continue;
    const int64_t r = long_rows[1 + 2 * i];
    const int len = row_start[r + 1] - row_start[r];
    if (len <= LONG_CHUNK) continue;
    const int nch = (len + LONG_CHUNK - 1) / LONG_CHUNK;
    float acc[VE], gsum[VE];
#pragma unroll
    for (int k = 0; k < VE; ++k) { acc[k] = 0.f; gsum[k] = 0.f; }
    constexpr int U = 8;
    int c = 0;
    for (; c + U <= nch; c += U) {
      float4 va[U][VE / 4], vg[U][VE / 4];
#pragma unroll
      for (int u = 0; u < U; ++u) {
        const float4* sa = reinterpret_cast<const float4*>(scratch + ((size_t)(i + c + u) * 2) * (L * VE) + lane_v * VE);
        const float4* sg = reinterpret_cast<const float4*>(scratch + ((size_t)(i + c + u) * 2 + 1) * (L * VE) + lane_v * VE);
#pragma unroll
        for (int k = 0; k < VE / 4; ++k) { va[u][k] = sa[k]; vg[u][k] = sg[k]; }
      }
#pragma unroll
      for (int u = 0; u < U; ++u)
#pragma unroll
        for (int k = 0; k < VE / 4; ++k) {
          acc[4 * k] += va[u][k].x; acc[4 * k + 1] += va[u][k].y; acc[4 * k + 2] += va[u][k].z; acc[4 * k + 3] += va[u][k].w;
          gsum[4 * k] += vg[u][k].x; gsum[4 * k + 1] += vg[u][k].y; gsum[4 * k + 2] += vg[u][k].z; gsum[4 * k + 3] += vg[u][k].w;
        }
    }
    for (; c < nch; ++c) {
      const float* sa = scratch + ((size_t)(i + c) * 2) * (L * VE) + lane_v * VE;
#pragma unroll
      for (int k = 0; k < VE; ++k) { acc[k] += sa[k]; gsum[k] += sa[L * VE + k]; }
    }
    if (HAS_FM && fm_sum != nullptr) {
      float w[VE];
      Vec16<T>::unpack(table[r * L + lane_v], w);
#pragma unroll
      for (int k = 0; k < VE; ++k) acc[k] = fmaf(-w[k], gsum[k], acc[k]);
    }
    sink_vec<T, RW, LOG2L>(sink, grad, sink_row(sink, r) * L + lane_v, acc, true);
  }
}

template <typename T>
__global__ __launch_bounds__(256) void build_tg_kernel(const uint4* __restrict__ g_fm, const float* __restrict__ fm_sum,
                                                       uint4* __restrict__ tg, int64_t B, int L) {
  constexpr int VE = Vec16<T>::VE;
  const int64_t total = B * L, stride = (int64_t)gridDim.x * blockDim.x;
  for (int64_t t = (int64_t)blockIdx.x * blockDim.x + threadIdx.x; t < total; t += stride) {
    const int64_t b = t / L;
    const int lv = (int)(t - b * L);
    const uint4 gv = g_fm[t];
    float g[VE], o[VE];
    Vec16<T>::unpack(gv, g);
    const float* sp = fm_sum + t * VE;
#pragma unroll
    for (int k = 0; k < VE; ++k) o[k] = g[k] * sp[k];
    tg[b * 2 * L + lv] = Vec16<T>::pack(o);
    tg[b * 2 * L + L + lv] = gv;
  }
}

template <typename T>
__global__ __launch_bounds__(256) void build_tg1_kernel(const T* __restrict__ g1, const float* __restrict__ fm_sum,
                                                        uint4* __restrict__ tg, uint4* __restrict__ gvec, int64_t B, int L) {
  constexpr int VE = Vec16<T>::VE;
  const int64_t total = B * L, stride = (int64_t)gridDim.x * blockDim.x;
  for (int64_t t = (int64_t)blockIdx.x * blockDim.x + threadIdx.x; t < total; t += stride) {
    const int64_t b = t / L;
    const float g = to_f32(g1[b]);
    float o[VE], gg[VE];
    const float* sp = fm_sum + t * VE;
#pragma unroll
    for (int k = 0; k < VE; ++k) { o[k] = g * sp[k]; gg[k] = g; }
    tg[t] = Vec16<T>::pack(o);
    if (t == b * L) gvec[b] = Vec16<T>::pack(gg);
  }
}

template <typename T>
__device__ __forceinline__ float elem_term(const T* __restrict__ g_rows, const T* __restrict__ g_fm,
                                           const float* __restrict__ fm_sum, int64_t p, int E, int N, int64_t gbs, int e,
                                           float* gsum, int gcols) {
  const int64_t b = p / N;
  float acc = 0.f;
  if (g_rows != nullptr) acc += to_f32(g_rows[(b * gbs + (p - b * N)) * E + e]);
  if (g_fm != nullptr) {
    const float gf = to_f32(g_fm[gcols == 1 ? b : b * E + e]);
    if (fm_sum != nullptr) {
      acc = fmaf(gf, fm_sum[b * E + e], acc);
      *gsum += gf;
    } else {
      acc += gf;
    }
  }
  return acc;
}

template <typename T>
__global__ __launch_bounds__(256) void scatter_rows_elem_kernel(
    const T* __restrict__ g_rows, const T* __restrict__ g_fm, const float* __restrict__ fm_sum,
    const T* __restrict__ table, const int32_t* __restrict__ row_start, const int32_t* __restrict__ perm, int64_t V,
    int E, int N, int64_t gbs, int64_t padding_row, T* __restrict__ grad, int32_t* __restrict__ long_rows,
    RowSink sink, int gcols, int32_t* __restrict__ split_rows ,
    float* __restrict__ split_acc ) {
  const int64_t total = V * E;
  const int64_t stride = (int64_t)gridDim.x * blockDim.x;
  const bool f32 = total < ((int64_t)1 << 32);
  for (int64_t t = (int64_t)blockIdx.x * blockDim.x + threadIdx.x; t < total; t += stride) {
    const int64_t r = udiv_fast(t, E, f32);
    const int e = (int)(t - r * E);
    float acc = 0.f, gsum = 0.f;
    bool touched = false;
    if (r != padding_row) {
      const int beg = row_start[r], end = row_start[r + 1];
      touched = end > beg;
      if (end - beg > ELEM_SPLIT) {
        if (e == 0) {
          const int nch = (end - beg + ELEM_SPLIT - 1) / ELEM_SPLIT;
// ... 77 lines not shown
#pragma unroll
        for (int u = 0; u < U; ++u) pp[u] = (q + 64 * u) < end ? perm[q + 64 * u] : -1;
#pragma unroll
        for (int u = 0; u < U; ++u)
          if (pp[u] >= 0) acc += elem_term<T>(g_rows, g_fm, fm_sum, pp[u], E, N, gbs, e, &gsum, gcols);
      }
#pragma unroll
      for (int m = 32; m >= 1; m >>= 1) {
        acc += __shfl_xor(acc, m, 64);
        gsum += __shfl_xor(gsum, m, 64);
      }
      if (lane == 0) {
        atomicAdd(&racc[e], acc);
        atomicAdd(&racc[E + e], gsum);
      }
    }
  }
}

template <typename T>
__global__ __launch_bounds__(256) void scatter_split_rows_finish_elem_kernel(
    const T* __restrict__ g_fm, const float* __restrict__ fm_sum, const T* __restrict__ table, int E,
    T* __restrict__ grad, const int32_t* __restrict__ split_rows, const float* __restrict__ split_acc, RowSink sink) {
  const int nent = split_rows[0];
  const int64_t total = (int64_t)nent * E;
  for (int64_t t = (int64_t)blockIdx.x * blockDim.x + threadIdx.x; t < total; t += (int64_t)gridDim.x * blockDim.x) {
    const int i = (int)(t / E), e = (int)(t - (int64_t)i * E);
    if (split_rows[2 + 2 * i] != 0) continue;
    const int64_t r = split_rows[1 + 2 * i];
    float acc = split_acc[(size_t)i * 2 * E + e];
    if (g_fm != nullptr && fm_sum != nullptr) acc = fmaf(-to_f32(table[r * E + e]), split_acc[(size_t)i * 2 * E + E + e], acc);
    sink_elem<T>(sink, grad, sink_row(sink, r) * E + e, acc, true);
  }
}

static const RowSink GRAD_SINK{0, 0.f, 0.f, nullptr};

struct WalkJob {
  const void* g_rows = nullptr;
  int64_t gbs = 0;
  const void* g_fm = nullptr;
  int g_fm_cols = 0;
  const float* fm_sum = nullptr;
  const void* table = nullptr;
  const int32_t* row_start = nullptr;
  const int32_t* perm = nullptr;
  int64_t B = 0, V = 0;
  int E = 0, N = 0;
  int64_t padding_row = -1;
  void* out = nullptr;
  const void* g_first = nullptr;
  void* grad_first = nullptr;
  int32_t* long_rows = nullptr;
  void* tg = nullptr;
  float* scratch = nullptr;
  RowSink sink = GRAD_SINK;
  hipStream_t s = nullptr;
  const char* who = "scatter_rows";
};

template <typename T, int LOG2L, bool RW>
static void scatter_group_launch(const WalkJob& j) {
  const int L = 1 << LOG2L;
  hipStream_t s = j.s;
  FmSrc fs{nullptr, nullptr, 0, 0};
  bool scal = false;
  const void* fm = j.g_fm;
  if (j.g_fm != nullptr && j.fm_sum != nullptr) {
    if (j.g_fm_cols == 1) {
      uint4* gvec = (uint4*)j.tg + j.B * L;
      hipLaunchKernelGGL((build_tg1_kernel<T>), dim3(stream_grid(j.B * L, 256, 4096)), dim3(256), 0, s,
                         (const T*)j.g_fm, j.fm_sum, (uint4*)j.tg, gvec, j.B, L);
      fs = FmSrc{(const uint4*)j.tg, gvec, L, 1};
      fs.g1 = j.g_fm;
      scal = j.g_first == nullptr;
    } else {
      hipLaunchKernelGGL((build_tg_kernel<T>), dim3(stream_grid(j.B * L, 256, 4096)), dim3(256), 0, s,
                         (const uint4*)j.g_fm, j.fm_sum, (uint4*)j.tg, j.B, L);
      fs = FmSrc{(const uint4*)j.tg, (const uint4*)j.tg + L, 2 * L, 2 * L};
    }
    fm = j.tg;
  }
  const int grid = stream_grid(j.V * L, 256, 256 * 32);
  const bool hg = j.g_rows != nullptr, hf = fm != nullptr;
#define TRS_SC_TAIL(HG, HF, SC)                                                                                 \
  do {                                                                                                          \
    hipLaunchKernelGGL((scatter_long_rows_kernel<T, LOG2L, HG, HF, SC, RW>), dim3(2048), dim3(256), 0, s,            \
                       (const uint4*)j.g_rows, (const uint4*)fm, j.fm_sum, (const uint4*)j.table, j.row_start,  \
                       j.perm, j.N, j.gbs, (uint4*)j.out, j.long_rows, j.scratch, j.sink, fs);                  \
    hipLaunchKernelGGL((scatter_long_rows_finish_kernel<T, LOG2L, HF, RW>), dim3(64), dim3(256), 0, s, j.fm_sum,    \
                       (const uint4*)j.table, j.row_start, (uint4*)j.out, j.long_rows, j.scratch, j.sink);      \
  } while (0)
#define TRS_SC(HG, HF)                                                                                          \
  do {                                                                                                          \
    if (j.g_first != nullptr)                                                                                   \
      hipLaunchKernelGGL((scatter_rows_group_kernel<T, LOG2L, HG, HF, true>), dim3(grid), dim3(256), 0, s,       \
                         (const uint4*)j.g_rows, (const uint4*)fm, j.fm_sum, (const uint4*)j.table, j.row_start, \
                         j.perm, j.V, j.N, j.gbs, j.padding_row, (uint4*)j.out, j.long_rows, j.sink, fs,        \
                         (const T*)j.g_first, (T*)j.grad_first);                                                \
    else                                                                                                        \
      hipLaunchKernelGGL((scatter_rows_group_kernel<T, LOG2L, HG, HF, false, false, 2, RW>), dim3(grid), dim3(256), 0, s,             \
                         (const uint4*)j.g_rows, (const uint4*)fm, j.fm_sum, (const uint4*)j.table, j.row_start, \
                         j.perm, j.V, j.N, j.gbs, j.padding_row, (uint4*)j.out, j.long_rows, j.sink, fs);       \
    TRS_SC_TAIL(HG, HF, false);                                                                                 \
  } while (0)
#define TRS_SCS(HG, CHF_)                                                                                       \
  do {                                                                                                          \
    hipLaunchKernelGGL((scatter_rows_group_kernel<T, LOG2L, HG, true, false, true, CHF_, RW>), dim3(grid), dim3(256), 0, s, \
                       (const uint4*)j.g_rows, (const uint4*)fm, j.fm_sum, (const uint4*)j.table, j.row_start,  \
                       j.perm, j.V, j.N, j.gbs, j.padding_row, (uint4*)j.out, j.long_rows, j.sink, fs);         \
    TRS_SC_TAIL(HG, true, true);                                                                                \
  } while (0)
  const bool lean = scal && (j.B * j.N) * (int64_t)L < ((int64_t)1 << 31) && j.V * (int64_t)L < ((int64_t)1 << 31) &&
                    j.N >= 2 && (j.B * j.N) * (int64_t)j.N < ((int64_t)1 << 32) && j.gbs == j.N;
  if (lean) {
    const unsigned rcpN = (unsigned)((((uint64_t)1 << 32) + (unsigned)j.N - 1) / (unsigned)j.N);
    if (hg)
      hipLaunchKernelGGL((scatter_rows_fm1_kernel<T, LOG2L, true, RW>), dim3(grid), dim3(256), 0, s, (const uint4*)j.g_rows,
                         (const uint4*)j.tg, (const T*)fs.g1, (const uint4*)j.table, j.row_start, j.perm, (int)j.V,
                         (unsigned)j.N, rcpN, (int)j.padding_row, (uint4*)j.out, j.long_rows, j.sink);
    else
      hipLaunchKernelGGL((scatter_rows_fm1_kernel<T, LOG2L, false, RW>), dim3(grid), dim3(256), 0, s, (const uint4*)j.g_rows,
                         (const uint4*)j.tg, (const T*)fs.g1, (const uint4*)j.table, j.row_start, j.perm, (int)j.V,
                         (unsigned)j.N, rcpN, (int)j.padding_row, (uint4*)j.out, j.long_rows, j.sink);
    if (hg) TRS_SC_TAIL(true, true, true);
    else TRS_SC_TAIL(false, true, true);
  } else if (scal) {
    if (hg) TRS_SCS(true, 2);
    else TRS_SCS(false, 2);
  } else if (hg && hf) TRS_SC(true, true);
  else if (hg) TRS_SC(true, false);
// ... 157 lines not shown
  }
  return check_launch("csr_build");
}

extern "C" int trs_csr_build(const void* idx, int32_t idx_dtype, const int64_t* offsets, int64_t B, int32_t N,
                             int64_t V, int32_t* row_start, int32_t* perm, void* workspace, size_t ws_bytes,
                             int32_t* err_flag, trs_stream_t stream) {
  return csr_build_impl(idx, idx_dtype, offsets, B, N, V, row_start, perm, workspace, ws_bytes, err_flag, stream, -1);
}

extern "C" int trs_csr_build_skip(const void* idx, int32_t idx_dtype, const int64_t* offsets, int64_t B, int32_t N,
                                  int64_t V, int64_t skip_row, int32_t* row_start, int32_t* perm, void* workspace,
                                  size_t ws_bytes, int32_t* err_flag, trs_stream_t stream) {
  TRS_REQUIRE(skip_row >= -1 && skip_row < V, TRS_EINVAL, "csr_build_skip: skip_row %lld outside [-1, V)",
              (long long)skip_row);
  return csr_build_impl(idx, idx_dtype, offsets, B, N, V, row_start, perm, workspace, ws_bytes, err_flag, stream,
                        skip_row);
}

static size_t long_row_entries(int64_t BN) { return (size_t)(BN / LONG_ROW + BN / LONG_CHUNK + 2); }
static size_t long_row_queue_bytes(int64_t BN) {
  return align_up(std::max(long_row_entries(BN) * 8 + 8,
                           (size_t)(BN / LONG_ROW_ELEM + 3) * 4 + (size_t)(BN / ELEM_SPLIT + BN / LONG_ROW_ELEM / 64 + 2) * 8 + 8),
                  256);
}

extern "C" size_t trs_scatter_workspace_bytes(int64_t BN, int32_t N, int32_t E, int32_t dtype) {
  const int64_t B = N > 0 ? (BN + N - 1) / N : 0;
  return long_row_queue_bytes(BN) + align_up((size_t)B * 2 * E * dtype_size(dtype), 256) +
         align_up(long_row_entries(BN) * 2 * E * 4, 256);
}

static int scatter_rows_impl(WalkJob j, int64_t BN, int32_t dtype, void* workspace, size_t ws_bytes) {
  TRS_REQUIRE(j.row_start && j.perm && j.out && workspace, TRS_EINVAL, "scatter_rows: NULL pointer");
  TRS_REQUIRE(j.g_rows || j.g_fm, TRS_EINVAL, "scatter_rows: need g_rows and/or g_fm");
  TRS_REQUIRE((j.fm_sum == nullptr) || (j.g_fm && j.table), TRS_EINVAL, "scatter_rows: fm_sum needs g_fm and table");
  TRS_REQUIRE(j.g_fm == nullptr || j.g_fm_cols == j.E || (j.g_fm_cols == 1 && j.fm_sum != nullptr), TRS_EINVAL,
              "scatter_rows: g_fm_cols %d (E = %d full rows, or 1 = constant along E with fm_sum)", j.g_fm_cols, j.E);
  if (j.gbs <= 0) j.gbs = j.N;
  TRS_REQUIRE(j.gbs >= j.N, TRS_EINVAL, "scatter_rows: g_rows_batch_stride %lld < N", (long long)j.gbs);
  TRS_REQUIRE(j.V > 0 && j.E > 0 && j.N > 0 && BN >= 0, TRS_EINVAL, "scatter_rows: bad size");
  TRS_REQUIRE(dtype == TRS_F32 || dtype == TRS_BF16, TRS_EDTYPE, "scatter_rows: dtype %d", dtype);
  TRS_REQUIRE(ws_bytes >= trs_scatter_workspace_bytes(BN, j.N, j.E, dtype), TRS_EWORKSPACE,
              "scatter_rows: workspace %zu < %zu", ws_bytes, trs_scatter_workspace_bytes(BN, j.N, j.E, dtype));
  TRS_REQUIRE(BN % j.N == 0, TRS_EINVAL, "scatter_rows: B*N=%lld not a multiple of N=%d", (long long)BN, j.N);
  const int lg = walk_lanes(j, dtype_size(dtype));
  TRS_REQUIRE(j.sink.mode != 4 || lg >= 0, TRS_ESHAPE,
              "%s: row-wise Adagrad needs rows of 1, 2, 4 .. 64 whole 16-byte vectors behind 16-byte aligned pointers "
              "(E = %d, %d bytes per value)", j.who, j.E, dtype_size(dtype));
  j.B = BN / j.N;
  j.long_rows = (int32_t*)workspace;
  j.tg = (char*)workspace + long_row_queue_bytes(BN);
  j.scratch = (float*)((char*)j.tg + align_up((size_t)j.B * 2 * j.E * dtype_size(dtype), 256));
  hipLaunchKernelGGL(zero_two_i32_kernel, dim3(1), dim3(64), 0, j.s, j.long_rows,
                     j.long_rows + 1 + (BN / LONG_ROW_ELEM + 2));
  return dtype == TRS_F32 ? scatter_launch<float>(j, lg) : scatter_launch<bf16_t>(j, lg);
}

extern "C" int trs_scatter_rows_first(const void* g_rows, int64_t g_rows_batch_stride, const void* g_fm, int32_t g_fm_cols,
                                      const float* fm_sum, const void* table, const int32_t* row_start,
                                      const int32_t* perm, int64_t BN, int64_t V, int32_t E, int32_t N, int32_t dtype,
                                      int64_t padding_row, void* grad_table, const void* g_first, void* grad_first,
                                      void* workspace, size_t ws_bytes, trs_stream_t stream) {
  TRS_REQUIRE(g_first && grad_first, TRS_EINVAL, "scatter_rows_first: NULL first-order pointer");
  return scatter_rows_impl(WalkJob{.g_rows = g_rows, .gbs = g_rows_batch_stride, .g_fm = g_fm, .g_fm_cols = g_fm_cols,
                                   .fm_sum = fm_sum, .table = table, .row_start = row_start, .perm = perm, .V = V, .E = E,
                                   .N = N, .padding_row = padding_row, .out = grad_table, .g_first = g_first,
                                   .grad_first = grad_first, .sink = GRAD_SINK, .s = (hipStream_t)stream},
                           BN, dtype, workspace, ws_bytes);
}

extern "C" int trs_scatter_rows(const void* g_rows, int64_t g_rows_batch_stride, const void* g_fm, int32_t g_fm_cols,
                                const float* fm_sum,
                                const void* table, const int32_t* row_start, const int32_t* perm, int64_t BN, int64_t V,
                                int32_t E, int32_t N, int32_t dtype, int64_t padding_row, void* grad_table,
                                void* workspace, size_t ws_bytes, trs_stream_t stream) {
  return scatter_rows_impl(WalkJob{.g_rows = g_rows, .gbs = g_rows_batch_stride, .g_fm = g_fm, .g_fm_cols = g_fm_cols,
                                   .fm_sum = fm_sum, .table = table, .row_start = row_start, .perm = perm, .V = V, .E = E,
                                   .N = N, .padding_row = padding_row, .out = grad_table, .sink = GRAD_SINK,
                                   .s = (hipStream_t)stream},
                           BN, dtype, workspace, ws_bytes);
}

static int make_sink(const char* who, const void* table, int32_t optimizer, float lr, const float* lr_dev, float eps,
                     float beta1, float beta2, float* state, float* state2, const int32_t* row_map, int64_t map_rows,
                     RowSink* sink) {
  TRS_REQUIRE(table, TRS_EINVAL, "%s: NULL table", who);
  const bool rowwise = optimizer == (2 | TRS_OPT_ROWWISE);
  TRS_REQUIRE((optimizer >= 1 && optimizer <= 3) || rowwise, TRS_EINVAL,
              "%s: optimizer %d (1 = SGD, 2 = Adagrad, 3 = Adam, 2 | TRS_OPT_ROWWISE = row-wise Adagrad)", who, optimizer);
  if (rowwise) {
    TRS_REQUIRE(state != nullptr, TRS_EINVAL, "%s: row-wise Adagrad needs the state buffer (V fp32)", who);
    *sink = RowSink{.mode = 4, .lr = lr, .eps = eps, .state = state, .row_map = row_map, .map_rows = map_rows,
                    .lr_dev = lr_dev};
    return TRS_OK;
  }
  TRS_REQUIRE(optimizer == 1 || state != nullptr, TRS_EINVAL, "%s: optimizer %d needs the state buffer", who, optimizer);
  TRS_REQUIRE(optimizer != 3 || state2 != nullptr, TRS_EINVAL, "%s: Adam needs both moments", who);
  TRS_REQUIRE(optimizer != 3 || (beta1 >= 0.f && beta1 < 1.f && beta2 >= 0.f && beta2 < 1.f), TRS_EINVAL,
              "%s: betas (%g, %g) must be in [0, 1)", who, (double)beta1, (double)beta2);
  *sink = RowSink{.mode = optimizer, .lr = lr, .eps = eps, .state = state, .beta1 = beta1, .beta2 = beta2,
                  .state2 = state2, .row_map = row_map, .map_rows = map_rows, .lr_dev = lr_dev};
  return TRS_OK;
}

extern "C" int trs_scatter_rows_update(const void* g_rows, int64_t g_rows_batch_stride, const void* g_fm, int32_t g_fm_cols,
                                       const float* fm_sum, void* table, const int32_t* row_start, const int32_t* perm,
                                       int64_t BN, int64_t V, int32_t E, int32_t N, int32_t dtype, int64_t padding_row,
// ... 51 lines not shown
```

torecsys_amd/functional.py:

```python
from __future__ import annotations

import ctypes
import os
from typing import List, Optional, Sequence, Tuple

import torch
from torch.autograd import Function
from torch.autograd.function import once_differentiable

from . import _abi
from ._abi import call, index_dtype_code, ptr, require_device, size_query, stream_ptr, value_dtype_code

CHECK_INDICES = os.environ.get("TRS_CHECK_INDICES", "0") not in ("", "0")


def _as_index(idx: torch.Tensor) -> torch.Tensor:
    idx = idx.rename(None) if idx.has_names() else idx
    if idx.dtype not in (torch.int64, torch.int32):
        if idx.dtype.is_floating_point or idx.dtype == torch.bool:
            raise TypeError(f"indices must be an integer tensor, got {idx.dtype}")
        idx = idx.long()
    return idx.contiguous()


# ... 2942 lines not shown

    def __enter__(self):
        global _mlp_family_request
        self.prev, _mlp_family_request = _mlp_family_request, self.request
        return self

    def __exit__(self, *exc):
        global _mlp_family_request
        _mlp_family_request = self.prev
        return False


def mlp_fused_family(widths: Sequence[int], rows: int, request: Optional[int] = None) -> int:
    req = _mlp_family_request if request is None else int(request)
    wl = _i32_array(widths)
    fam = int(_abi.load().trs_mlp_fused_family(len(widths) - 1, wl, int(rows), req))
    if fam == 0 and req != MLP_FAMILY_AUTO:
        fam = int(_abi.load().trs_mlp_fused_family(len(widths) - 1, wl, int(rows), MLP_FAMILY_AUTO))
    if fam == 0:
        raise RuntimeError(f"torecsys_amd: no fused-MLP kernel family for widths {list(widths)}")
    return fam


def fused_mlp_forward_raw(x2: torch.Tensor, Ws: Sequence[torch.Tensor], bs: Sequence[torch.Tensor],
                          input_mask: bool = False, family: Optional[int] = None, x_stride: int = 0):
    L = len(Ws)
    widths = [Ws[0].shape[1]] + [w.shape[0] for w in Ws]
    rows, dev = x2.shape[0], x2.device
    if x_stride and (x_stride < widths[0] or x2.shape[1] != x_stride or not x2.is_contiguous()):
        raise ValueError(f"fused_mlp_forward_raw: x_stride {x_stride} does not describe x2 {tuple(x2.shape)}")
    fam = mlp_fused_family(widths, rows, family)
    hidden = [torch.empty(rows, _pad32(widths[l + 1]), dtype=torch.bfloat16, device=dev) for l in range(L - 1)]
    mask_bytes = size_query("trs_mlp_fused_mask_bytes", rows)
    masks = [torch.empty(mask_bytes, dtype=torch.uint8, device=dev) for _ in range(L - 1)]
    mask_in = torch.empty(mask_bytes, dtype=torch.uint8, device=dev) if input_mask else None
    y = torch.empty(rows, widths[L], dtype=torch.bfloat16, device=dev)
    wl = _i32_array(widths)
    ws_bytes = size_query("trs_mlp_fused_workspace_bytes", L, wl)
    ws = torch.empty(ws_bytes, dtype=torch.uint8, device=dev)
    call("trs_mlp_fused_fwd", ptr(x2), rows, L, wl, _ptr_array(Ws), _ptr_array(bs), _ptr_array(hidden),
         _ptr_array(masks), ptr(mask_in), ptr(y), _abi.TRS_BF16, fam, int(x_stride), ptr(ws), ws_bytes, stream_ptr())
    if input_mask:
        return y, hidden, masks, mask_in, fam
    return y, hidden, masks, fam


def mlp_bwd_wlast_bytes(widths: Sequence[int], rows: int, family: int, live: int) -> int:
    return size_query("trs_mlp_fused_bwd_wlast_part_bytes", len(widths) - 1, _i32_array(widths), int(rows), _abi.TRS_BF16,
                      int(family), int(live))


def fused_mlp_backward_raw(gy2: torch.Tensor, widths: Sequence[int], Ws: Sequence[torch.Tensor],
                           masks: Sequence[torch.Tensor], mask_in: Optional[torch.Tensor] = None, *, family: int,
                           h_last: Optional[torch.Tensor] = None, live: int = 0):
    if family not in (MLP_FAMILY_TILE, MLP_FAMILY_ROW_OWNER, MLP_FAMILY_MIXED):
        raise ValueError("fused_mlp_backward_raw: family must be the value the forward returned with these masks")
    L = len(Ws)
    rows, dev = gy2.shape[0], gy2.device
    gz = [torch.empty(rows, _pad32(widths[l + 1]), dtype=torch.bfloat16, device=dev) for l in range(L - 1)]
    gb = [torch.empty(_pad32(widths[l + 1]), dtype=torch.float32, device=dev) for l in range(L)]
    gx = torch.empty(rows, widths[0], dtype=torch.bfloat16, device=dev)
    gb_in = torch.empty(_pad32(widths[0]), dtype=torch.float32, device=dev) if mask_in is not None else None
    wl = _i32_array(widths)
    ws_bytes = size_query("trs_mlp_fused_workspace_bytes", L, wl)
    ws = torch.empty(ws_bytes, dtype=torch.uint8, device=dev)
    if h_last is not None:
        if not (gy2.is_contiguous() and h_last.is_contiguous() and h_last.shape[0] == rows):
            raise ValueError("fused_mlp_backward_raw: gy2 / h_last must be contiguous over the same rows")
        part_bytes = mlp_bwd_wlast_bytes(widths, max(rows, 1), family, live)
        part = torch.empty(max(part_bytes, 16), dtype=torch.uint8, device=dev)
        gw_last = torch.empty(live, _pad32(widths[L - 1]), dtype=torch.float32, device=dev)
        call("trs_mlp_fused_bwd_data_wlast", ptr(gy2), gy2.shape[1], rows, L, wl, _ptr_array(Ws), _ptr_array(masks),
             _ptr_array(gz), _ptr_array(gb), ptr(gx), ptr(mask_in), ptr(gb_in), ptr(h_last), h_last.shape[1], int(live),
             ptr(part), part_bytes, ptr(gw_last), _abi.TRS_BF16, int(family), ptr(ws), ws_bytes, stream_ptr())
        return gx, gz, gb, gb_in, gw_last
    call("trs_mlp_fused_bwd_data", ptr(gy2), rows, L, wl, _ptr_array(Ws), _ptr_array(masks), _ptr_array(gz),
         _ptr_array(gb), ptr(gx), ptr(mask_in), ptr(gb_in), _abi.TRS_BF16, int(family), ptr(ws), ws_bytes, stream_ptr())
    return gx, gz, gb, gb_in


class _FusedMLP(Function):

    @staticmethod
    def forward(ctx, x, *params):
        require_device(x, *params)
        L = len(params) // 2
        Ws = [params[2 * l].contiguous() for l in range(L)]
        bs = [params[2 * l + 1].contiguous() for l in range(L)]
        widths = [Ws[0].shape[1]] + [w.shape[0] for w in Ws]
        x2 = x.reshape(-1, widths[0]).contiguous()
        y, hidden, masks, fam = fused_mlp_forward_raw(x2, Ws, bs)
        ctx.save_for_backward(x2, *Ws, *hidden, *masks)
        ctx.meta = (L, widths, tuple(x.shape), [p.dtype for p in params], fam)
        return y.reshape(*x.shape[:-1], widths[L])

    @staticmethod
    @once_differentiable
    def backward(ctx, gy):
        L, widths, xshape, pdt, fam = ctx.meta
        saved = ctx.saved_tensors
        x2, Ws = saved[0], saved[1:1 + L]
        hidden, masks = saved[1 + L:L + L], saved[L + L:]
        rows, dev = x2.shape[0], x2.device
        gy2 = gy.reshape(rows, widths[L]).contiguous()
        same_dt = all(pdt[2 * l] == pdt[2 * l + 1] for l in range(L))
        gw_last = None
        if (same_dt and ctx.needs_input_grad[2 * L - 1] and gy2.dtype == torch.bfloat16
                and mlp_bwd_wlast_bytes(widths, rows, fam, widths[L]) > 0):
            gx, gz, gb, _, gw_last = fused_mlp_backward_raw(gy2, widths, Ws, masks, family=fam, h_last=hidden[L - 2],
                                                            live=widths[L])
        else:
            gx, gz, gb, _ = fused_mlp_backward_raw(gy2, widths, Ws, masks, family=fam)
        grads = []
        if same_dt:
            for gw, gbias in _tail_grads([(gy2 if l == L - 1 else gz[l], x2 if l == 0 else hidden[l - 1], widths[l + 1],
                                           widths[l], pdt[2 * l], gb[l], ctx.needs_input_grad[1 + 2 * l],
                                           ctx.needs_input_grad[2 + 2 * l]) for l in range(L)], gw_last):
                grads += [gw, gbias]
            return (gx.reshape(xshape) if ctx.needs_input_grad[0] else None, *grads)
        for l in range(L):
            inp = x2 if l == 0 else hidden[l - 1]
            g = gy2 if l == L - 1 else gz[l]
            need_w, need_b = ctx.needs_input_grad[1 + 2 * l], ctx.needs_input_grad[2 + 2 * l]
            if pdt[2 * l] == pdt[2 * l + 1]:
                gw, gbias = _tail_layer_grads(g, inp, widths[l + 1], widths[l], pdt[2 * l], gb[l], need_w, need_b)
            else:
                gw = _wgrad_rows(g, inp, widths[l + 1], widths[l], pdt[2 * l]) if need_w else None
                gbias = gb[l][:widths[l + 1]].to(pdt[2 * l + 1]) if need_b else None
            grads += [gw, gbias]
        return (gx.reshape(xshape) if ctx.needs_input_grad[0] else None, *grads)

# ... 16 lines not shown


def rows_gemm(g: torch.Tensor, W: torch.Tensor, out_f: int, in_f: int) -> torch.Tensor:
    y = torch.empty(g.shape[0], in_f, dtype=torch.bfloat16, device=g.device)
    ws_bytes = size_query("trs_rows_gemm_workspace_bytes", out_f, in_f)
    ws = torch.empty(ws_bytes, dtype=torch.uint8, device=g.device)
    call("trs_rows_gemm", ptr(g), g.shape[0], g.shape[1], ptr(W), out_f, in_f, _abi.TRS_BF16, ptr(y), ptr(ws), ws_bytes,
         stream_ptr())
    return y


def _tail_layer_grads(g, inp, out_f, in_f, dtype, gb_f32, need_w, need_b):
    if need_w and need_b:
        return _wgrad_rows(g, inp, out_f, in_f, dtype, gb_f32)
    gw = _wgrad_rows(g, inp, out_f, in_f, dtype) if need_w else None
    return gw, (gb_f32[:out_f].to(dtype) if need_b else None)


def _wgrad_many_splits(jobs) -> int:
    if not WGRAD_ROWS or len(jobs) < 2:
        return 0
    for g, inp, _, _ in jobs:
        if not (g.is_cuda and g.dtype == torch.bfloat16 and inp.dtype == torch.bfloat16 and g.is_contiguous()
                and inp.is_contiguous() and g.shape[0] == jobs[0][0].shape[0]):
            return 0
    return size_query("trs_wgrad_rows_many_splits", len(jobs), _i32_array([j[2] for j in jobs]),
                      _i32_array([j[3] for j in jobs]), _i32_array([j[0].shape[1] for j in jobs]),
                      _i32_array([j[1].shape[1] for j in jobs]), int(jobs[0][0].shape[0]))


DEEP_WGRAD_MIN_ROWS = 16384


def _wgrad_deep_jobs(first, tail):
    jobs = []
    for g, inp, out_f, in_f, dtype, gb_f32, _, need_b in [first] + tail:
        M_x, N_g = (in_f + 207) // 208 * 208, (out_f + 15) // 16 * 16
        if not (g.is_cuda and g.dtype == inp.dtype == dtype == torch.bfloat16 and g.dim() == inp.dim() == 2
                and g.is_contiguous() and inp.is_contiguous() and g.shape[0] == inp.shape[0] == first[0].shape[0]
                and M_x <= inp.shape[1] and N_g <= g.shape[1] and (not need_b or gb_f32 is not None)):
            return None
        jobs.append((inp, g, M_x, N_g, out_f, in_f, gb_f32 if need_b else None))
    return jobs


def _wgrad_deep_splits(jobs) -> int:
    if not WGRAD_ROWS or jobs is None or not 2 <= len(jobs) <= 4 or jobs[0][0].shape[0] < DEEP_WGRAD_MIN_ROWS:
        return 0
    return size_query("trs_wgrad_wide_many_splits", len(jobs), _i32_array([j[2] for j in jobs]),
                      _i32_array([j[0].shape[1] for j in jobs]), _i32_array([j[3] for j in jobs]),
                      _i32_array([j[1].shape[1] for j in jobs]), int(jobs[0][0].shape[0]))


def _wgrad_deep(jobs, S, casts):
    dev, rows = jobs[0][0].device, int(jobs[0][0].shape[0])
    parts = [torch.empty(S, j[2], j[3], dtype=torch.float32, device=dev) for j in jobs]
    call("trs_wgrad_wide_many", len(jobs), _ptr_array([j[0] for j in jobs]), _i32_array([j[0].shape[1] for j in jobs]),
         _ptr_array([j[1] for j in jobs]), _i32_array([j[1].shape[1] for j in jobs]), rows,
         _i32_array([j[2] for j in jobs]), _i32_array([j[3] for j in jobs]), S, _ptr_array(parts), stream_ptr())
    gws = [torch.empty(j[4], j[5], dtype=torch.bfloat16, device=dev) for j in jobs]
    gbs = [torch.empty(j[4], dtype=torch.bfloat16, device=dev) if j[6] is not None else None for j in jobs]
    n = len(casts)
    call("trs_wgrad_finish_t_many", len(jobs) + n, _ptr_array(parts + [None] * n), S,
         _i32_array([j[2] for j in jobs] + [0] * n), _i32_array([j[3] for j in jobs] + [0] * n),
         _i32_array([j[4] for j in jobs] + [0] * n), _i32_array([j[5] for j in jobs] + [c[0] for c in casts]),
         _abi.TRS_BF16, _ptr_array(gws + [None] * n), _ptr_array([j[6] for j in jobs] + [c[1] for c in casts]),
         _ptr_array(gbs + [c[2] for c in casts]), stream_ptr())
    return list(zip(gws, gbs))


def _tail_grads(layers, gw_last=None, first=None):
    out = [None] * len(layers)
    batch = [k for k, t in enumerate(layers[:-1]) if t[6]]
    deep = _wgrad_deep_jobs(first, [layers[k] for k in batch]) if first is not None and first[6] and batch else None
    S_deep = _wgrad_deep_splits(deep)
    jobs = [(layers[k][0], layers[k][1], min(layers[k][0].shape[1], (layers[k][2] + 7) // 8 * 8),
             min(layers[k][1].shape[1], (layers[k][3] + 7) // 8 * 8)) for k in batch]
    S = _wgrad_many_splits(jobs) if S_deep == 0 and len({layers[k][4] for k in batch}) == 1 else 0
    casts = []
    if gw_last is not None:
        _, _, out_f, in_f, dt, gb_f32, _, need_b = layers[-1]
        gw = torch.empty(out_f, in_f, dtype=dt, device=gw_last.device)
        gbias = torch.empty(out_f, dtype=dt, device=gw_last.device) if need_b else None
        casts = [(in_f, gw_last[r], gw[r]) for r in range(out_f)] + ([(out_f, gb_f32, gbias)] if need_b else [])
        out[-1] = (gw, gbias)

    def finish(parts, S, R, Cc, orows, ocols, gws, gbfs, gbs, dtype_code, extra):
        n = len(extra)
        call("trs_wgrad_finish_many", len(parts) + n, _ptr_array(parts + [None] * n), S, _i32_array(R + [0] * n),
             _i32_array(Cc + [0] * n), _i32_array(orows + [0] * n), _i32_array(ocols + [c[0] for c in extra]), dtype_code,
             _ptr_array(gws + [None] * n), _ptr_array(gbfs + [c[1] for c in extra]), _ptr_array(gbs + [c[2] for c in extra]),
             stream_ptr())

    first_out = None
    if S_deep > 0:
        ride_casts = casts if casts and layers[-1][4] == torch.bfloat16 and len(deep) + len(casts) <= 8 else []
        first_out, *rest = _wgrad_deep(deep, S_deep, ride_casts)
        if ride_casts:
            casts = []
        for k, gwb in zip(batch, rest):
            out[k] = gwb
    if S > 0:
        dev, dtype, rows = jobs[0][0].device, layers[batch[0]][4], jobs[0][0].shape[0]
        parts = [torch.empty(S, M, N, dtype=torch.float32, device=dev) for _, _, M, N in jobs]
        call("trs_wgrad_rows_many", len(jobs), _ptr_array([j[0] for j in jobs]), _i32_array([j[0].shape[1] for j in jobs]),
             _ptr_array([j[1] for j in jobs]), _i32_array([j[1].shape[1] for j in jobs]), rows,
             _i32_array([j[2] for j in jobs]), _i32_array([j[3] for j in jobs]), S, _ptr_array(parts), stream_ptr())
        gws, gbs, gbfs = [], [], []
        for k in batch:
            _, _, out_f, in_f, _, gb_f32, _, need_b = layers[k]
            gws.append(torch.empty(out_f, in_f, dtype=dtype, device=dev))
            ride = need_b and out_f <= (in_f + 255) // 256 * 256
            gbs.append(torch.empty(out_f, dtype=dtype, device=dev) if ride else None)
            gbfs.append(gb_f32 if ride else None)
        ride_casts = casts if casts and layers[-1][4] == dtype and len(jobs) + len(casts) <= 8 else []
        finish(parts, S, [j[2] for j in jobs], [j[3] for j in jobs], [layers[k][2] for k in batch],
               [layers[k][3] for k in batch], gws, gbfs, gbs, value_dtype_code(gws[0]), ride_casts)
        if ride_casts:
            casts = []
        for n, k in enumerate(batch):
            gb = gbs[n]
            if gb is None and layers[k][7]:
                gb = layers[k][5][:layers[k][2]].to(dtype)
            out[k] = (gws[n], gb)
    if casts:
        finish([], 1, [], [], [], [], [], [], [], value_dtype_code(casts[0][2]), casts)
    for k, t in enumerate(layers):
        if out[k] is None:
            out[k] = _tail_layer_grads(*t)
    return out if first is None else out + [first_out]


WGRAD_ROWS = os.environ.get("TRS_WGRAD_ROWS", "1") not in ("", "0")


def pad_cols(g: torch.Tensor, width: int) -> torch.Tensor:
    g = g.contiguous()
    out = torch.empty(g.shape[0], width, dtype=g.dtype, device=g.device)
    call("trs_pad_cols", ptr(g), g.shape[1], ptr(out), width, g.shape[0], value_dtype_code(g), stream_ptr())
    return out


def _wgrad_rows(g: torch.Tensor, inp: torch.Tensor, out_f: int, in_f: int, dtype, gb_f32: Optional[torch.Tensor] = None):
    if gb_f32 is not None:
        gb = torch.empty(out_f, dtype=dtype, device=g.device)
        if out_f <= (in_f + 255) // 256 * 256:
            return _wgrad_rows_impl(g, inp, out_f, in_f, dtype, gb_f32, gb), gb
        gb.copy_(gb_f32[:out_f])
        return _wgrad_rows_impl(g, inp, out_f, in_f, dtype, None, None), gb
    return _wgrad_rows_impl(g, inp, out_f, in_f, dtype, None, None)


def _wgrad_rows_impl(g, inp, out_f, in_f, dtype, gb_f32, gb):
    rows = g.shape[0]
    if (WGRAD_ROWS and g.is_cuda and g.dtype == torch.bfloat16 and inp.dtype == torch.bfloat16 and g.is_contiguous()
            and inp.is_contiguous()):
        M, N = min(g.shape[1], (out_f + 7) // 8 * 8), min(inp.shape[1], (in_f + 7) // 8 * 8)
        S = int(_abi.load().trs_wgrad_rows_splits(M, N, int(rows)))
        if S > 0:
            part = torch.empty(S, M, N, dtype=torch.float32, device=g.device)
            call("trs_wgrad_rows", ptr(g), g.shape[1], ptr(inp), inp.shape[1], rows, M, N,
                 _abi.TRS_BF16, S, ptr(part), stream_ptr())
            gw = torch.empty(out_f, in_f, dtype=dtype, device=g.device)
            call("trs_wgrad_finish", ptr(part), S, M, N, out_f, in_f, value_dtype_code(gw),
                 ptr(gw), ptr(gb_f32), ptr(gb), stream_ptr())
            return gw
    S = 0
    for cand in (192, 128, 96, 64, 48, 32, 24, 16, 12, 8, 6, 4):
        if rows % cand == 0 and rows // cand >= 1024:
            S = cand
            break
    if S == 0:
        if gb is not None:
            gb.copy_(gb_f32[:out_f])
        return (g.t() @ inp)[:out_f, :in_f].contiguous().to(dtype)
    part = torch.bmm(g.view(S, rows // S, -1).transpose(1, 2), inp.view(S, rows // S, -1), out_dtype=torch.float32)
    gw = torch.empty(out_f, in_f, dtype=dtype, device=g.device)
    call("trs_wgrad_finish", ptr(part), S, part.shape[1], part.shape[2], out_f, in_f, value_dtype_code(gw), ptr(gw),
         ptr(gb_f32), ptr(gb), stream_ptr())
    return gw


# ... 400 lines not shown
```

torecsys_amd/layers.py:

```python
from __future__ import annotations

from abc import ABC, abstractmethod
from typing import Dict, List, Optional, Tuple

import math
import os

import torch
import torch.nn as nn

from . import functional as F_


def _strip(t: torch.Tensor) -> torch.Tensor:
    return t.rename(None) if t.has_names() else t


class BaseLayer(nn.Module, ABC):

    def __init__(self, **kwargs):
        super().__init__()

    @property
    @abstractmethod
# ... 647 lines not shown

def _dense_layer_grads(g2, gbf, xin, W, out_f, in_f, wdt, need_x, need_w, need_b, done=None):
    rows = xin.shape[0]
    gw_out = gb_out = None
    S = _split_count(rows, _LinearSplitK.SPLIT_ROWS)
    if done is not None:
        gw_out, gb_out = done
    elif need_w or (need_b and gbf is not None):
        Sw = _wide_wgrad_splits(g2, xin, out_f, in_f) if need_w else 0
        if Sw:
            gw = torch.empty(out_f, in_f, dtype=wdt, device=xin.device)
            part = torch.empty(Sw, in_f, out_f, dtype=torch.float32, device=xin.device)
            F_.call("trs_wgrad_wide", F_.ptr(xin), xin.stride(0), F_.ptr(g2), g2.stride(0), rows, in_f, out_f, Sw,
                    F_.ptr(part), F_.stream_ptr())
            with_b = need_b and gbf is not None
            gb = torch.empty(out_f, dtype=wdt, device=xin.device) if with_b else None
            F_.call("trs_wgrad_finish_t", F_.ptr(part), Sw, in_f, out_f, out_f, in_f, F_.value_dtype_code(gw),
                    F_.ptr(gw), F_.ptr(gbf) if with_b else F_.ptr(None), F_.ptr(gb), F_.stream_ptr())
            gw_out = gw
            if with_b:
                gb_out = gb
        elif need_w and S >= 4 and rows % S == 0 and 32 <= g2.shape[1] <= 1024 and 32 <= xin.shape[1] <= 4096 \
                and xin.is_contiguous():
            gw = torch.empty(out_f, in_f, dtype=wdt, device=xin.device)
            St = _split_count(rows, _MLPStack.SPLIT_ROWS_WIDE)
            if xin.shape[1] >= 2 * g2.shape[1] and St >= 4:
                part = torch.bmm(xin.view(St, rows // St, -1).transpose(1, 2), g2.view(St, rows // St, -1),
                                 out_dtype=torch.float32)
                with_b = need_b and gbf is not None
                gb = torch.empty(out_f, dtype=wdt, device=xin.device) if with_b else None
                F_.call("trs_wgrad_finish_t", F_.ptr(part), St, part.shape[1], part.shape[2], out_f, in_f,
                        F_.value_dtype_code(gw), F_.ptr(gw), F_.ptr(gbf) if with_b else F_.ptr(None), F_.ptr(gb),
                        F_.stream_ptr())
            else:
                part = torch.bmm(g2.view(S, rows // S, -1).transpose(1, 2), xin.view(S, rows // S, -1),
                                 out_dtype=torch.float32)
                with_b = need_b and gbf is not None and out_f <= (in_f + 255) // 256 * 256
                gb = torch.empty(out_f, dtype=wdt, device=xin.device) if with_b else None
                F_.call("trs_wgrad_finish", F_.ptr(part), S, part.shape[1], part.shape[2], out_f, in_f,
                        F_.value_dtype_code(gw), F_.ptr(gw), F_.ptr(gbf) if with_b else F_.ptr(None), F_.ptr(gb),
                        F_.stream_ptr())
            gw_out = gw
            if with_b:
                gb_out = gb
        elif need_w:
            gw = (g2.t() @ xin)[:out_f, :in_f]
            gw_out = gw if gw.is_contiguous() else gw.contiguous()
    if need_b and gb_out is None:
        gb_out = gbf[:out_f].to(wdt) if gbf is not None else g2.sum(0)[:out_f]
    gx = None
    if need_x and F_.rows_gemm_supported(g2, W, out_f, xin.shape[1]) and W.shape[1] == xin.shape[1]:
        gx = F_.rows_gemm(g2, W, out_f, xin.shape[1])
    elif need_x:
        gx = g2 @ W
    return gx, gw_out, gb_out


class _HybridMLP(torch.autograd.Function):

    @staticmethod
    def forward(ctx, x, w_narrow, *tensors):
        cur = x.reshape(-1, x.shape[-1])
        w1, b1, w1u, b1u = tensors[:4]
        tail = tensors[4:]
        W1 = w1 if w1u is None else w1u
        B1 = b1 if w1u is None else b1u
        L = len(tail) // 4
        Ws = [(tail[4 * l] if tail[4 * l + 2] is None else tail[4 * l + 2]).contiguous() for l in range(L)]
        bs = [(tail[4 * l + 1] if tail[4 * l + 3] is None else tail[4 * l + 3]).contiguous() for l in range(L)]
        h1 = torch._addmm_activation(B1, cur, W1.t(), use_gelu=False)
        if w_narrow is not None:
            y, hidden, masks, mask_in, fam = F_.fused_mlp_forward_raw(h1, [w_narrow] + Ws[1:], bs, input_mask=True,
                                                                      family=F_.MLP_FAMILY_MIXED, x_stride=h1.shape[1])
        else:
            y, hidden, masks, mask_in, fam = F_.fused_mlp_forward_raw(h1, Ws, bs, input_mask=True)
        out_f = tail[4 * (L - 1)].shape[0]
        ctx.save_for_backward(cur, W1, h1, mask_in, *Ws, *hidden, *masks)
        ctx.meta = (L, [h1.shape[1]] + [w.shape[0] for w in Ws], [tuple(tail[4 * l].shape) for l in range(L)],
                    [tail[4 * l].dtype for l in range(L)], tuple(w1.shape), w1.dtype, tuple(x.shape), fam)
        y = y[:, :out_f] if out_f != y.shape[1] else y
        return y.reshape(*x.shape[:-1], out_f)

    @staticmethod
    @torch.autograd.function.once_differentiable
    def backward(ctx, gy):
        L, widths, wshapes, wdt, w1shape, w1dt, xshape, fam = ctx.meta
        saved = ctx.saved_tensors
        cur, W1, h1, mask_in = saved[:4]
        Ws = saved[4:4 + L]
        hidden, masks = saved[4 + L:3 + L + L], saved[3 + L + L:]
        needs = ctx.needs_input_grad
        gy = gy.reshape(h1.shape[0], -1)
        live, gw_last = wshapes[L - 1][0], None
        if (needs[6 + 4 * (L - 1)] and gy.dtype == torch.bfloat16 and gy.shape[1] == live
                and F_.mlp_bwd_wlast_bytes(widths, h1.shape[0], fam, live) > 0):
            gy2 = gy.contiguous()
            g1, gz, gb, gb1, gw_last = F_.fused_mlp_backward_raw(gy2, widths, Ws, masks, mask_in, family=fam,
                                                                 h_last=hidden[L - 2], live=live)
        else:
            gy2 = F_.pad_cols(gy, widths[L]) if gy.shape[1] != widths[L] else gy.contiguous()
            g1, gz, gb, gb1 = F_.fused_mlp_backward_raw(gy2, widths, Ws, masks, mask_in, family=fam)
        grads = []
        *tail, done = F_._tail_grads([(gy2 if l == L - 1 else gz[l], h1 if l == 0 else hidden[l - 1], *wshapes[l],
                                       wdt[l], gb[l], needs[6 + 4 * l], needs[7 + 4 * l]) for l in range(L)], gw_last,
                                     first=(g1, cur, w1shape[0], w1shape[1], w1dt, gb1, needs[2], needs[3]))
        for gw, gbias in tail:
            grads += [gw, gbias, None, None]
        gx, gw1, gbias1 = _dense_layer_grads(g1, gb1, cur, W1, w1shape[0], w1shape[1], w1dt, needs[0], needs[2], needs[3],
                                             done)
        return (gx.reshape(xshape) if needs[0] else None, None, gw1, gbias1, None, None, *grads)


class _MLPStack(torch.autograd.Function):

    SPLIT_ROWS_WIDE = 4096

    @staticmethod
    def forward(ctx, x, spec, *tensors):
        cur = x.reshape(-1, x.shape[-1])
        saved, wmeta = [], []
        for l, (fuse, rowdot) in enumerate(spec):
            weight, bias, w_use, b_use = tensors[4 * l:4 * l + 4]
            W = weight if w_use is None else w_use
            Bv = bias if w_use is None else b_use
            if rowdot:
                Wf = W.reshape(-1)
                out = torch.empty(cur.shape[0], 1, dtype=cur.dtype, device=cur.device)
                F_.call("trs_rowdot_fwd", F_.ptr(cur), F_.ptr(Wf), F_.ptr(Bv), cur.shape[0], cur.shape[1],
                        F_.value_dtype_code(cur), F_.ptr(out), F_.stream_ptr())
                W = Wf
            elif fuse:
                out = torch._addmm_activation(Bv, cur, W.t(), use_gelu=False)
            else:
                out = torch.addmm(Bv, cur, W.t())
            saved += [cur, W, out if fuse else None]
            wmeta.append((tuple(weight.shape), weight.dtype))
            cur = out
        ctx.spec, ctx.wmeta, ctx.xshape = spec, wmeta, tuple(x.shape)
        ctx.save_for_backward(*saved)
        return cur.reshape(*x.shape[:-1], cur.shape[-1])

    @staticmethod
    @torch.autograd.function.once_differentiable
    def backward(ctx, g):
        saved, spec = ctx.saved_tensors, ctx.spec
        needs = ctx.needs_input_grad
        grads = [None] * (4 * len(spec))
        g2 = g.reshape(-1, g.shape[-1])
        if not g2.is_contiguous():
            g2 = g2.contiguous()
        for l in range(len(spec) - 1, -1, -1):
            xin, W, y = saved[3 * l:3 * l + 3]
            fuse, rowdot = spec[l]
            (out_f, in_f), wdt = ctx.wmeta[l]
            need_x = l > 0 or needs[0]
            need_w, need_b = needs[2 + 4 * l], needs[3 + 4 * l]
            rows = xin.shape[0]
            if rowdot:
                C = xin.shape[1]
                gh = torch.empty_like(xin) if need_x else None
# ... 433 lines not shown
```

Measured before the change: 66.98 million samples/s.

## Fold MLP bias-gradient partial sums into the weight-gradient finish kernels

Adds a backward-data entry point that leaves per-block column partial sums for the bias gradients unreduced. The existing wgrad finish kernels gain a parts mode that folds those partials while they cast the bias outputs. The goal is to drop the separate bias-reduction pass and its launch from the fused MLP backward. The merged path only runs when the bf16 and family conditions hold; otherwise it falls back to an explicit colsum reduce. It also saves the narrow first weight for backward, which changes the widths metadata.

```diff
diff --git a/include/trs_abi.h b/include/trs_abi.h
--- a/include/trs_abi.h
+++ b/include/trs_abi.h
@@ -236,6 +236,13 @@
                                  const void* h_last, int32_t h_stride, int32_t live, float* wl_part,
                                  size_t wl_part_bytes, float* gw_last, int32_t dtype, int32_t family, void* workspace,
                                  size_t ws_bytes, trs_stream_t stream);
+int trs_mlp_fused_bwd_data_parts(const void* gy, int32_t gy_stride, int64_t rows, int32_t num_layers,
+                                 const int32_t* widths, const void* const* weights, const void* const* masks,
+                                 void* const* gz, void* gx, const void* mask_in, const void* h_last, int32_t h_stride,
+                                 int32_t live, float* wl_part, size_t wl_part_bytes, const float** part_out, int32_t* stride_out, int32_t* nparts_out, int32_t dtype,
+                                 int32_t family, void* workspace, size_t ws_bytes, trs_stream_t stream);
+int trs_colsum_parts_reduce(int32_t n_sets, const float* const* part, const int32_t* stride, const int32_t* n,
+                            int32_t nparts, float* const* out, trs_stream_t stream);
 
 int trs_pad_cols(const void* src, int32_t c_in, void* dst, int32_t c_out, int64_t rows, int32_t dtype,
                  trs_stream_t stream);
@@ -316,6 +323,14 @@
 int trs_wgrad_finish_t_many(int32_t n_jobs, const float* const* part, int32_t S, const int32_t* Cc, const int32_t* R,
                             const int32_t* out_rows, const int32_t* out_cols, int32_t dtype, void* const* gw,
                             const float* const* gb_f32, void* const* gb, trs_stream_t stream);
+int trs_wgrad_finish_many_parts(int32_t n_jobs, const float* const* part, int32_t S, const int32_t* R, const int32_t* Cc,
+                                const int32_t* out_rows, const int32_t* out_cols, int32_t dtype, void* const* gw,
+                                const float* const* gb_f32, void* const* gb, const int32_t* gb_nparts,
+                                const int32_t* gb_stride, trs_stream_t stream);
+int trs_wgrad_finish_t_many_parts(int32_t n_jobs, const float* const* part, int32_t S, const int32_t* Cc, const int32_t* R,
+                                  const int32_t* out_rows, const int32_t* out_cols, int32_t dtype, void* const* gw,
+                                  const float* const* gb_f32, void* const* gb, const int32_t* gb_nparts,
+                                  const int32_t* gb_stride, trs_stream_t stream);
 int trs_copy_padded_many(const int64_t* desc, int32_t n, int32_t elem_size, int64_t max_elems, trs_stream_t stream);
 
 int32_t trs_cin_glue_blocks(int64_t B);
diff --git a/torecsys_amd/_abi.py b/torecsys_amd/_abi.py
--- a/torecsys_amd/_abi.py
+++ b/torecsys_amd/_abi.py
@@ -41,6 +41,8 @@
     "trs_wgrad_wide_many_map": (c_int32, [_I32, _P, _P, _P, _P, _I64, _I32, _P]),
     "trs_wgrad_wide_many": (c_int32, [_I32, _P, _P, _P, _P, _I64, _P, _P, _I32, _P, _P]),
     "trs_wgrad_finish_t_many": (c_int32, [_I32, _P, _I32, _P, _P, _P, _P, _I32, _P, _P, _P, _P]),
+    "trs_wgrad_finish_many_parts": (c_int32, [_I32, _P, _I32, _P, _P, _P, _P, _I32, _P, _P, _P, _P, _P, _P]),
+    "trs_wgrad_finish_t_many_parts": (c_int32, [_I32, _P, _I32, _P, _P, _P, _P, _I32, _P, _P, _P, _P, _P, _P]),
     "trs_copy_padded_many":(c_int32, [_P, _I32, _I32, _I64, _P]),
     "trs_cin_glue_blocks": (c_int32, [_I64]),
     "trs_cin_glue_stats": (c_int32, [_P, _I64, _I32, _I32, _I32, _P, _P]),
@@ -190,6 +192,9 @@
     "trs_mlp_fused_bwd_wlast_part_bytes": (_SZ, [_I32, _P, _I64, _I32, _I32, _I32]),
     "trs_mlp_fused_bwd_data_wlast": (c_int32, [_P, _I32, _I64, _I32, _P, _P, _P, _P, _P, _P, _P, _P, _P, _I32, _I32, _P, _SZ, _P,
                                                _I32, _I32, _P, _SZ, _P]),
+    "trs_mlp_fused_bwd_data_parts": (c_int32, [_P, _I32, _I64, _I32, _P, _P, _P, _P, _P, _P, _P, _I32, _I32, _P, _SZ, _P, _P,
+                                               _P, _I32, _I32, _P, _SZ, _P]),
+    "trs_colsum_parts_reduce": (c_int32, [_I32, _P, _P, _P, _I32, _P, _P]),
     "trs_ctr_logit_fwd": (c_int32, [_P, _I32, _P, _I32, _P, _P, _I32, _P, _I64, _I32, _P, _P]),
     "trs_bce_logits_workspace_bytes": (_SZ, [_I64]),
     "trs_bce_logits_fwd": (c_int32, [_P, _I32, _P, _I32, _I64, _P, _P, _SZ, _P]),
@@ -348,18 +353,23 @@
     return out
 
 
+_TIMED_AS = {"trs_wgrad_finish_many_parts": "trs_wgrad_finish_many",
+             "trs_wgrad_finish_t_many_parts": "trs_wgrad_finish_t_many"}
+
+
 def call(name: str, *args):
-    rec = _timed.get(name)
+    timed_as = _TIMED_AS.get(name, name)
+    rec = _timed.get(timed_as)
     if rec is not None:
         st = stream_ptr()
         if torch.cuda.is_current_stream_capturing():
-            ring = _mark_ring(name)
+            ring = _mark_ring(timed_as)
             lib = load()
             lib.trs_mark_timestamp(ctypes.c_void_p(ring.data_ptr()), _MARK_CAP, st)
             rc = getattr(lib, name)(*args)
             lib.trs_mark_timestamp(ctypes.c_void_p(ring.data_ptr()), _MARK_CAP, st)
         else:
-            ev = _every[name]
+            ev = _every[timed_as]
             ev[1] += 1
             if ev[1] % ev[0] == 0:
                 a, b = _HipEvent(), _HipEvent()
diff --git a/torecsys_amd/csrc/mlp_epilogue.hip b/torecsys_amd/csrc/mlp_epilogue.hip
--- a/torecsys_amd/csrc/mlp_epilogue.hip
+++ b/torecsys_amd/csrc/mlp_epilogue.hip
@@ -234,12 +234,38 @@
 }
 
 template <typename T>
+__device__ __forceinline__ void wf_fold(const float* __restrict__ gbf, int nparts, int pstride, int c0, int count, int limit,
+                                        T* __restrict__ out) {
+  __shared__ float red[16][17];
+  const int cl = threadIdx.x & 15, w = threadIdx.x >> 4;
+  for (int base = c0; base < c0 + count && base < limit; base += 16) {
+    const int c = base + cl;
+    const bool live = c < c0 + count && c < limit;
+    float s = 0.f;
+    if (live) {
+#pragma unroll 4
+      for (int p = w; p < nparts; p += 16) s += gbf[(size_t)p * pstride + c];
+    }
+    red[w][cl] = s;
+    __syncthreads();
+    if (w == 0 && live) {
+      float t = 0.f;
+#pragma unroll
+      for (int k = 0; k < 16; ++k) t += red[k][cl];
+      out[c] = from_f32<T>(t);
+    }
+    __syncthreads();
+  }
+}
+
+template <typename T>
 __device__ __forceinline__ void wgrad_finish_body(const float* __restrict__ part, int S, int R, int Cc, int out_rows,
                                                   int out_cols, T* __restrict__ gw, const float* __restrict__ gbf,
-                                                  T* __restrict__ gb) {
+                                                  T* __restrict__ gb, int nparts = 0, int pstride = 0) {
   const int c = blockIdx.x * 256 + threadIdx.x;
   if ((int)blockIdx.y == out_rows) {
-    if (gb != nullptr && c < out_rows) gb[c] = from_f32<T>(gbf[c]);
+    if (gb != nullptr && nparts > 0) wf_fold<T>(gbf, nparts, pstride, blockIdx.x * 256, 256, out_rows, gb);
+    else if (gb != nullptr && c < out_rows) gb[c] = from_f32<T>(gbf[c]);
     return;
   }
   if ((int)blockIdx.y > out_rows || c >= out_cols) return;
@@ -272,6 +298,7 @@
   const float* gbf;
   void* gb;
   int R, Cc, out_rows, out_cols;
+  int nparts, pstride;
 };
 struct WgradFinishArgs {
   WgradFinishJob job[WF_MAXJ];
@@ -282,10 +309,12 @@
   const WgradFinishJob& j = a.job[blockIdx.z];
   if (j.part == nullptr) {
     const int c = blockIdx.x * 256 + threadIdx.x;
-    if (blockIdx.y == 0 && c < j.out_cols) ((T*)j.gb)[c] = from_f32<T>(j.gbf[c]);
+    if (j.nparts > 0)
+      wf_fold<T>(j.gbf, j.nparts, j.pstride, (blockIdx.y * gridDim.x + blockIdx.x) * 16, 16, j.out_cols, (T*)j.gb);
+    else if (blockIdx.y == 0 && c < j.out_cols) ((T*)j.gb)[c] = from_f32<T>(j.gbf[c]);
     return;
   }
-  wgrad_finish_body<T>(j.part, a.S, j.R, j.Cc, j.out_rows, j.out_cols, (T*)j.gw, j.gbf, (T*)j.gb);
+  wgrad_finish_body<T>(j.part, a.S, j.R, j.Cc, j.out_rows, j.out_cols, (T*)j.gw, j.gbf, (T*)j.gb, j.nparts, j.pstride);
 }
 
 constexpr int WF_SL = 16;
@@ -329,12 +358,13 @@
 template <typename T>
 __device__ __forceinline__ void wgrad_finish_t_body(const float* __restrict__ part, int S, int Cc, int R, int out_rows,
                                                     int out_cols, T* __restrict__ gw, const float* __restrict__ gbf,
-                                                    T* __restrict__ gb) {
+                                                    T* __restrict__ gb, int nparts = 0, int pstride = 0) {
   __shared__ float tile[32][33];
   const int tx = threadIdx.x & 31, ty = threadIdx.x >> 5;
   if ((int)blockIdx.y == (out_cols + 31) / 32) {
     const int r = blockIdx.x * 32 + tx;
-    if (gb != nullptr && ty == 0 && r < out_rows) gb[r] = from_f32<T>(gbf[r]);
+    if (gb != nullptr && nparts > 0) wf_fold<T>(gbf, nparts, pstride, blockIdx.x * 32, 32, out_rows, gb);
+    else if (gb != nullptr && ty == 0 && r < out_rows) gb[r] = from_f32<T>(gbf[r]);
     return;
   }
   const int r0 = blockIdx.x * 32, c0 = blockIdx.y * 32;
@@ -377,11 +407,13 @@
   const WgradFinishJob& j = a.job[blockIdx.z];
   if (j.part == nullptr) {
     const int c = (blockIdx.y * gridDim.x + blockIdx.x) * 256 + threadIdx.x;
-    if (c < j.out_cols) ((T*)j.gb)[c] = from_f32<T>(j.gbf[c]);
+    if (j.nparts > 0)
+      wf_fold<T>(j.gbf, j.nparts, j.pstride, (blockIdx.y * gridDim.x + blockIdx.x) * 16, 16, j.out_cols, (T*)j.gb);
+    else if (c < j.out_cols) ((T*)j.gb)[c] = from_f32<T>(j.gbf[c]);
     return;
   }
   if ((int)blockIdx.x >= (j.out_rows + 31) / 32 || (int)blockIdx.y > (j.out_cols + 31) / 32) return;
-  wgrad_finish_t_body<T>(j.part, a.S, j.Cc, j.R, j.out_rows, j.out_cols, (T*)j.gw, j.gbf, (T*)j.gb);
+  wgrad_finish_t_body<T>(j.part, a.S, j.Cc, j.R, j.out_rows, j.out_cols, (T*)j.gw, j.gbf, (T*)j.gb, j.nparts, j.pstride);
 }
 
 }
@@ -733,9 +765,18 @@
   return check_launch("wgrad_finish");
 }
 
-extern "C" int trs_wgrad_finish_many(int32_t n_jobs, const float* const* part, int32_t S, const int32_t* R,
-                                     const int32_t* Cc, const int32_t* out_rows, const int32_t* out_cols, int32_t dtype,
-                                     void* const* gw, const float* const* gb_f32, void* const* gb, trs_stream_t stream) {
+static int wgrad_finish_parts_ok(const char* who, int k, const float* gbf, int cols, const int32_t* gb_nparts,
+                                 const int32_t* gb_stride) {
+  if (gb_nparts == nullptr || gb_nparts[k] == 0) return TRS_OK;
+  TRS_REQUIRE(gbf != nullptr && gb_nparts[k] > 0 && gb_stride[k] >= cols, TRS_EINVAL,
+              "%s: job %d: %d partial rows, %d floats apart, for %d columns", who, k, gb_nparts[k], gb_stride[k], cols);
+  return TRS_OK;
+}
+
+static int wgrad_finish_many_impl(int32_t n_jobs, const float* const* part, int32_t S, const int32_t* R,
+                                  const int32_t* Cc, const int32_t* out_rows, const int32_t* out_cols, int32_t dtype,
+                                  void* const* gw, const float* const* gb_f32, void* const* gb, const int32_t* gb_nparts,
+                                  const int32_t* gb_stride, trs_stream_t stream) {
   TRS_REQUIRE(n_jobs >= 1 && n_jobs <= WF_MAXJ, TRS_EINVAL, "wgrad_finish_many: %d jobs (1 .. %d)", n_jobs, WF_MAXJ);
   TRS_REQUIRE(part && R && Cc && out_rows && out_cols && gw && gb_f32 && gb, TRS_EINVAL, "wgrad_finish_many: NULL array");
   TRS_REQUIRE(S > 0, TRS_EINVAL, "wgrad_finish_many: bad size");
@@ -747,7 +788,9 @@
     if (part[k] == nullptr) {
       TRS_REQUIRE(gw[k] == nullptr && gb[k] && gb_f32[k] && out_cols[k] > 0, TRS_EINVAL,
                   "wgrad_finish_many: a job without a product takes gb_f32, gb and out_cols only (job %d)", k);
-      a.job[k] = WgradFinishJob{nullptr, nullptr, gb_f32[k], gb[k], 0, 0, 0, out_cols[k]};
+      if (int rc = wgrad_finish_parts_ok("wgrad_finish_many", k, gb_f32[k], out_cols[k], gb_nparts, gb_stride)) return rc;
+      a.job[k] = WgradFinishJob{nullptr, nullptr, gb_f32[k], gb[k], 0, 0, 0, out_cols[k], gb_nparts ? gb_nparts[k] : 0,
+                                gb_nparts ? gb_stride[k] : 0};
       max_cols = std::max(max_cols, out_cols[k]);
       continue;
     }
@@ -757,16 +800,38 @@
     TRS_REQUIRE((gb[k] == nullptr) == (gb_f32[k] == nullptr), TRS_EINVAL, "wgrad_finish_many: gb and gb_f32 go together (job %d)", k);
     TRS_REQUIRE(gb[k] == nullptr || out_rows[k] <= ((out_cols[k] + 255) / 256) * 256, TRS_ESHAPE,
                 "wgrad_finish_many: out_rows %d exceeds the bias row of workgroups", out_rows[k]);
-    a.job[k] = WgradFinishJob{part[k], gw[k], gb_f32[k], gb[k], R[k], Cc[k], out_rows[k], out_cols[k]};
+    if (int rc = wgrad_finish_parts_ok("wgrad_finish_many", k, gb_f32[k], out_rows[k], gb_nparts, gb_stride)) return rc;
+    a.job[k] = WgradFinishJob{part[k], gw[k], gb_f32[k], gb[k], R[k], Cc[k], out_rows[k], out_cols[k],
+                              gb_nparts ? gb_nparts[k] : 0, gb_nparts ? gb_stride[k] : 0};
     max_rows = std::max(max_rows, out_rows[k]);
     max_cols = std::max(max_cols, out_cols[k]);
   }
+  for (int k = 0; k < n_jobs; ++k)
+    if (part[k] == nullptr && a.job[k].nparts > 0) {
+      const int gx = (max_cols + 255) / 256, need = (out_cols[k] + 15) / 16;
+      if (gx * (max_rows + 1) < need) max_rows = (need + gx - 1) / gx - 1;
+    }
   dim3 grid((max_cols + 255) / 256, max_rows + 1, n_jobs);
   if (dtype == TRS_F32)
     hipLaunchKernelGGL((wgrad_finish_many_kernel<float>), grid, dim3(256), 0, (hipStream_t)stream, a);
   else
     hipLaunchKernelGGL((wgrad_finish_many_kernel<bf16_t>), grid, dim3(256), 0, (hipStream_t)stream, a);
   return check_launch("wgrad_finish_many");
+}
+
+extern "C" int trs_wgrad_finish_many(int32_t n_jobs, const float* const* part, int32_t S, const int32_t* R,
+                                     const int32_t* Cc, const int32_t* out_rows, const int32_t* out_cols, int32_t dtype,
+                                     void* const* gw, const float* const* gb_f32, void* const* gb, trs_stream_t stream) {
+  return wgrad_finish_many_impl(n_jobs, part, S, R, Cc, out_rows, out_cols, dtype, gw, gb_f32, gb, nullptr, nullptr, stream);
+}
+
+extern "C" int trs_wgrad_finish_many_parts(int32_t n_jobs, const float* const* part, int32_t S, const int32_t* R,
+                                           const int32_t* Cc, const int32_t* out_rows, const int32_t* out_cols,
+                                           int32_t dtype, void* const* gw, const float* const* gb_f32, void* const* gb,
+                                           const int32_t* gb_nparts, const int32_t* gb_stride, trs_stream_t stream) {
+  TRS_REQUIRE(gb_nparts && gb_stride, TRS_EINVAL, "wgrad_finish_many_parts: NULL array");
+  return wgrad_finish_many_impl(n_jobs, part, S, R, Cc, out_rows, out_cols, dtype, gw, gb_f32, gb, gb_nparts, gb_stride,
+                                stream);
 }
 
 extern "C" int trs_wgrad_finish_t(const float* part, int32_t S, int32_t Cc, int32_t R, int32_t out_rows, int32_t out_cols,
@@ -787,9 +852,10 @@
   return check_launch("wgrad_finish_t");
 }
 
-extern "C" int trs_wgrad_finish_t_many(int32_t n_jobs, const float* const* part, int32_t S, const int32_t* Cc,
-                                       const int32_t* R, const int32_t* out_rows, const int32_t* out_cols, int32_t dtype,
-                                       void* const* gw, const float* const* gb_f32, void* const* gb, trs_stream_t stream) {
+static int wgrad_finish_t_many_impl(int32_t n_jobs, const float* const* part, int32_t S, const int32_t* Cc,
+                                    const int32_t* R, const int32_t* out_rows, const int32_t* out_cols, int32_t dtype,
+                                    void* const* gw, const float* const* gb_f32, void* const* gb, const int32_t* gb_nparts,
+                                    const int32_t* gb_stride, trs_stream_t stream) {
   TRS_REQUIRE(n_jobs >= 1 && n_jobs <= WF_MAXJ, TRS_EINVAL, "wgrad_finish_t_many: %d jobs (1 .. %d)", n_jobs, WF_MAXJ);
   TRS_REQUIRE(part && R && Cc && out_rows && out_cols && gw && gb_f32 && gb, TRS_EINVAL, "wgrad_finish_t_many: NULL array");
   TRS_REQUIRE(S > 0, TRS_EINVAL, "wgrad_finish_t_many: bad size");
@@ -801,25 +867,48 @@
     if (part[k] == nullptr) {
       TRS_REQUIRE(gw[k] == nullptr && gb[k] && gb_f32[k] && out_cols[k] > 0, TRS_EINVAL,
                   "wgrad_finish_t_many: a job without a product takes gb_f32, gb and out_cols only (job %d)", k);
-      a.job[k] = WgradFinishJob{nullptr, nullptr, gb_f32[k], gb[k], 0, 0, 0, out_cols[k]};
+      if (int rc = wgrad_finish_parts_ok("wgrad_finish_t_many", k, gb_f32[k], out_cols[k], gb_nparts, gb_stride)) return rc;
+      a.job[k] = WgradFinishJob{nullptr, nullptr, gb_f32[k], gb[k], 0, 0, 0, out_cols[k], gb_nparts ? gb_nparts[k] : 0,
+                                gb_nparts ? gb_stride[k] : 0};
       continue;
     }
     TRS_REQUIRE(R[k] > 0 && Cc[k] > 0 && out_rows[k] > 0 && out_cols[k] > 0 && out_rows[k] <= R[k] && out_cols[k] <= Cc[k],
                 TRS_EINVAL, "wgrad_finish_t_many: bad size (job %d)", k);
     TRS_REQUIRE(part[k] && gw[k], TRS_EINVAL, "wgrad_finish_t_many: NULL pointer (job %d)", k);
     TRS_REQUIRE((gb[k] == nullptr) == (gb_f32[k] == nullptr), TRS_EINVAL, "wgrad_finish_t_many: gb and gb_f32 go together (job %d)", k);
-    a.job[k] = WgradFinishJob{part[k], gw[k], gb_f32[k], gb[k], R[k], Cc[k], out_rows[k], out_cols[k]};
+    if (int rc = wgrad_finish_parts_ok("wgrad_finish_t_many", k, gb_f32[k], out_rows[k], gb_nparts, gb_stride)) return rc;
+    a.job[k] = WgradFinishJob{part[k], gw[k], gb_f32[k], gb[k], R[k], Cc[k], out_rows[k], out_cols[k],
+                              gb_nparts ? gb_nparts[k] : 0, gb_nparts ? gb_stride[k] : 0};
     gx = std::max(gx, (out_rows[k] + 31) / 32);
     gy = std::max(gy, (out_cols[k] + 31) / 32 + 1);
   }
   for (int k = 0; k < n_jobs; ++k)
-    if (part[k] == nullptr && (out_cols[k] + 255) / 256 > gx * gy) gx = ((out_cols[k] + 255) / 256 + gy - 1) / gy;
+    if (part[k] == nullptr) {
+      const int need = a.job[k].nparts > 0 ? (out_cols[k] + 15) / 16 : (out_cols[k] + 255) / 256;
+      if (need > gx * gy) gx = (need + gy - 1) / gy;
+    }
   dim3 grid(gx, gy, n_jobs);
   if (dtype == TRS_F32)
     hipLaunchKernelGGL((wgrad_finish_t_many_kernel<float>), grid, dim3(256), 0, (hipStream_t)stream, a);
   else
     hipLaunchKernelGGL((wgrad_finish_t_many_kernel<bf16_t>), grid, dim3(256), 0, (hipStream_t)stream, a);
   return check_launch("wgrad_finish_t_many");
+}
+
+extern "C" int trs_wgrad_finish_t_many(int32_t n_jobs, const float* const* part, int32_t S, const int32_t* Cc,
+                                       const int32_t* R, const int32_t* out_rows, const int32_t* out_cols, int32_t dtype,
+                                       void* const* gw, const float* const* gb_f32, void* const* gb, trs_stream_t stream) {
+  return wgrad_finish_t_many_impl(n_jobs, part, S, Cc, R, out_rows, out_cols, dtype, gw, gb_f32, gb, nullptr, nullptr,
+                                  stream);
+}
+
+extern "C" int trs_wgrad_finish_t_many_parts(int32_t n_jobs, const float* const* part, int32_t S, const int32_t* Cc,
+                                             const int32_t* R, const int32_t* out_rows, const int32_t* out_cols,
+                                             int32_t dtype, void* const* gw, const float* const* gb_f32, void* const* gb,
+                                             const int32_t* gb_nparts, const int32_t* gb_stride, trs_stream_t stream) {
+  TRS_REQUIRE(gb_nparts && gb_stride, TRS_EINVAL, "wgrad_finish_t_many_parts: NULL array");
+  return wgrad_finish_t_many_impl(n_jobs, part, S, Cc, R, out_rows, out_cols, dtype, gw, gb_f32, gb, gb_nparts, gb_stride,
+                                  stream);
 }
 
 namespace trs {
diff --git a/torecsys_amd/csrc/mlp_fused.hip b/torecsys_amd/csrc/mlp_fused.hip
--- a/torecsys_amd/csrc/mlp_fused.hip
+++ b/torecsys_amd/csrc/mlp_fused.hip
@@ -946,6 +946,11 @@
   float* part;
   float* gw;
 };
+struct MlpBwdForm {
+  const float** part;
+  int32_t* stride;
+  int32_t* nparts;
+};
 static size_t mlp_bwd_lds(int L, const int32_t* widths, int live) {
   return (size_t)MF_ROWS * mlp_act_str(L, widths) + 8 * 512 * 4 + (size_t)(L + 1 + live) * 512 * 4;
 }
@@ -955,11 +960,12 @@
 static int mlp_fused_bwd_impl(const void* gy, int64_t rows, int32_t num_layers, const int32_t* widths,
                               const void* const* weights, const void* const* masks, void* const* gz,
                               float* const* gbias, void* gx, const void* mask_in, float* gbias_in, int32_t dtype,
-                              int32_t family, void* workspace, size_t ws_bytes, trs_stream_t stream, const MlpWlast* wl) {
+                              int32_t family, void* workspace, size_t ws_bytes, trs_stream_t stream, const MlpWlast* wl,
+                              const MlpBwdForm* form = nullptr) {
   hipStream_t s = (hipStream_t)stream;
   TRS_REQUIRE(dtype == TRS_BF16, TRS_EDTYPE, "mlp_fused_bwd_data: bf16 only");
   TRS_REQUIRE(trs_mlp_fused_supported(num_layers, widths), TRS_ESHAPE, "mlp_fused_bwd_data: unsupported layer widths");
-  TRS_REQUIRE(weights && workspace && gy && masks && gz && gbias, TRS_EINVAL, "mlp_fused_bwd_data: NULL pointer");
+  TRS_REQUIRE(weights && workspace && gy && masks && gz && (gbias || form), TRS_EINVAL, "mlp_fused_bwd_data: NULL pointer");
   TRS_REQUIRE(ws_bytes >= trs_mlp_fused_workspace_bytes(num_layers, widths), TRS_EWORKSPACE,
               "mlp_fused_bwd_data: workspace too small");
   const int L = num_layers;
@@ -976,7 +982,10 @@
   TRS_REQUIRE(fam_ok, TRS_EINVAL,
               "mlp_fused_bwd_data: family must be the TILE / ROW_OWNER / MIXED value the forward ran under (got %d)", family);
   TRS_REQUIRE(family != TRS_MLP_FAMILY_ROW_OWNER || gx != nullptr, TRS_EINVAL, "mlp_fused_bwd_data: the row-owner kernels need gx");
-  TRS_REQUIRE((mask_in == nullptr) == (gbias_in == nullptr) && (mask_in == nullptr || (L + 1 <= MF_MAXL && gx != nullptr)),
+  TRS_REQUIRE(form == nullptr || (rows > 0 && family != TRS_MLP_FAMILY_ROW_OWNER), TRS_EINVAL,
+              "mlp_fused_bwd_data_parts: the tile backward on at least one row only (family %d, %lld rows)", family, (long long)rows);
+  TRS_REQUIRE((form != nullptr || (mask_in == nullptr) == (gbias_in == nullptr)) &&
+                  (mask_in == nullptr || (L + 1 <= MF_MAXL && gx != nullptr)),
               TRS_EINVAL, "mlp_fused_bwd_data: mask_in and gbias_in come together (and with gx, at most %d layers)", MF_MAXL - 1);
   if (rows == 0) {
     for (int l = 0; l < L; ++l)
@@ -1053,6 +1062,22 @@
   auto* kern = a.ro_masks ? (wl ? mlp_fused_bwd_wlast_kernel<true> : mlp_fused_bwd_kernel<true>)
                           : (wl ? mlp_fused_bwd_wlast_kernel<false> : mlp_fused_bwd_kernel<false>);
   hipLaunchKernelGGL(kern, dim3(grid), dim3(64 * MF_WAVES), lds, s, a);
+  if (form != nullptr) {
+    for (int sidx = 0; sidx < L; ++sidx) {
+      const int l = L - 1 - sidx;
+      form->part[l] = a.step[sidx].colsum;
+      form->stride[l] = a.step[sidx].K;
+    }
+    form->part[L] = a.colsum_in;
+    form->stride[L] = a.colsum_in != nullptr ? pad32(widths[0]) : 0;
+    for (int j = 0; j < MF_MAXLIVE; ++j) {
+      const int Kh = pad32(widths[L - 1]);
+      form->part[L + 1 + j] = j < a.live ? wl->part + (size_t)j * Kh : nullptr;
+      form->stride[L + 1 + j] = j < a.live ? a.live * Kh : 0;
+    }
+    *form->nparts = grid;
+    return check_launch("mlp_fused_bwd_data_parts");
+  }
   MlpColsumArgs cs;
   cs.nparts = grid;
   int kmax = 0;
@@ -1175,3 +1200,57 @@
   hipLaunchKernelGGL(mlp_rows_gemm_kernel, dim3((int)std::min<int64_t>(ntiles, MF_GRID)), dim3(64 * MF_WAVES), lds, s, a);
   return check_launch("rows_gemm");
 }
+
+extern "C" int trs_mlp_fused_bwd_data_parts(const void* gy, int32_t gy_stride, int64_t rows, int32_t num_layers,
+                                            const int32_t* widths, const void* const* weights, const void* const* masks,
+                                            void* const* gz, void* gx, const void* mask_in, const void* h_last,
+                                            int32_t h_stride, int32_t live, float* wl_part, size_t wl_part_bytes,
+                                            const float** part_out, int32_t* stride_out, int32_t* nparts_out,
+                                            int32_t dtype, int32_t family, void* workspace, size_t ws_bytes,
+                                            trs_stream_t stream) {
+  const char* who = "mlp_fused_bwd_data_parts";
+  TRS_REQUIRE(dtype == TRS_BF16, TRS_EDTYPE, "%s: bf16 only", who);
+  TRS_REQUIRE(widths && num_layers >= 1 && num_layers <= MF_MAXL, TRS_EINVAL, "%s: bad stack", who);
+  TRS_REQUIRE(part_out && stride_out && nparts_out, TRS_EINVAL, "%s: NULL result array", who);
+  TRS_REQUIRE(rows > 0, TRS_EINVAL, "%s: no rows, no partials (trs_mlp_fused_bwd_data zero-fills)", who);
+  TRS_REQUIRE(family == TRS_MLP_FAMILY_TILE || family == TRS_MLP_FAMILY_MIXED, TRS_EINVAL,
+              "%s: the tile backward only (family %d)", who, family);
+  MlpWlast wl{nullptr, 0, 0, 0, nullptr, nullptr};
+  if (h_last != nullptr) {
+    TRS_REQUIRE(wl_part, TRS_EINVAL, "%s: NULL pointer", who);
+    const size_t need = trs_mlp_fused_bwd_wlast_part_bytes(num_layers, widths, rows, dtype, family, live);
+    TRS_REQUIRE(need > 0, TRS_ESHAPE, "%s: the output layer's dW is not carried for this stack / family %d / %d live columns",
+                who, family, live);
+    TRS_REQUIRE(wl_part_bytes >= need, TRS_EWORKSPACE, "%s: partial buffer too small", who);
+    TRS_REQUIRE(gy_stride == widths[num_layers] || (gy_stride == live && live < 8), TRS_ESHAPE,
+                "%s: gy_stride %d (widths[L] = %d, or the %d live columns alone)", who, gy_stride, widths[num_layers], live);
+    TRS_REQUIRE(h_stride >= pad32(widths[num_layers - 1]) && h_stride % 8 == 0, TRS_ESHAPE, "%s: h_stride %d", who, h_stride);
+    TRS_REQUIRE(aligned16(h_last) && aligned16(wl_part), TRS_EALIGN, "%s: 16-byte alignment", who);
+    wl = MlpWlast{h_last, h_stride, live, gy_stride, wl_part, nullptr};
+  } else {
+    TRS_REQUIRE(gy_stride == widths[num_layers], TRS_ESHAPE, "%s: gy_stride %d (widths[L] = %d)", who, gy_stride,
+                widths[num_layers]);
+  }
+  const MlpBwdForm form{part_out, stride_out, nparts_out};
+  return mlp_fused_bwd_impl(gy, rows, num_layers, widths, weights, masks, gz, nullptr, gx, mask_in, nullptr, dtype, family,
+                            workspace, ws_bytes, stream, h_last != nullptr ? &wl : nullptr, &form);
+}
+
+extern "C" int trs_colsum_parts_reduce(int32_t n_sets, const float* const* part, const int32_t* stride, const int32_t* n,
+                                       int32_t nparts, float* const* out, trs_stream_t stream) {
+  TRS_REQUIRE(n_sets >= 1 && n_sets <= MF_MAXL && part && stride && n && out && nparts > 0, TRS_EINVAL,
+              "colsum_parts_reduce: %d sets (1 .. %d) of %d partials", n_sets, MF_MAXL, nparts);
+  MlpColsumArgs cs;
+  cs.nparts = nparts;
+  int kmax = 0;
+  for (int k = 0; k < n_sets; ++k) {
+    TRS_REQUIRE(part[k] && out[k] && n[k] > 0 && stride[k] >= n[k], TRS_EINVAL, "colsum_parts_reduce: bad set %d", k);
+    cs.part[k] = part[k];
+    cs.out[k] = out[k];
+    cs.n[k] = n[k];
+    cs.stride[k] = stride[k];
+    kmax = std::max(kmax, n[k]);
+  }
+  hipLaunchKernelGGL(mlp_colsum_reduce_many_kernel, dim3((kmax + 63) / 64, n_sets), dim3(1024), 0, (hipStream_t)stream, cs);
+  return check_launch("colsum_parts_reduce");
+}
diff --git a/torecsys_amd/csrc/scatter.hip b/torecsys_amd/csrc/scatter.hip
--- a/torecsys_amd/csrc/scatter.hip
+++ b/torecsys_amd/csrc/scatter.hip
@@ -847,8 +847,10 @@
 
 template <typename T>
 __global__ __launch_bounds__(256) void build_tg_kernel(const uint4* __restrict__ g_fm, const float* __restrict__ fm_sum,
-                                                       uint4* __restrict__ tg, int64_t B, int L) {
+                                                       uint4* __restrict__ tg, int64_t B, int L,
+                                                       int32_t* __restrict__ zero_a, int32_t* __restrict__ zero_b) {
   constexpr int VE = Vec16<T>::VE;
+  if (zero_a != nullptr && blockIdx.x == 0 && threadIdx.x == 0) { *zero_a = 0; *zero_b = 0; }
   const int64_t total = B * L, stride = (int64_t)gridDim.x * blockDim.x;
   for (int64_t t = (int64_t)blockIdx.x * blockDim.x + threadIdx.x; t < total; t += stride) {
     const int64_t b = t / L;
@@ -866,8 +868,10 @@
 
 template <typename T>
 __global__ __launch_bounds__(256) void build_tg1_kernel(const T* __restrict__ g1, const float* __restrict__ fm_sum,
-                                                        uint4* __restrict__ tg, uint4* __restrict__ gvec, int64_t B, int L) {
+                                                        uint4* __restrict__ tg, uint4* __restrict__ gvec, int64_t B, int L,
+                                                        int32_t* __restrict__ zero_a, int32_t* __restrict__ zero_b) {
   constexpr int VE = Vec16<T>::VE;
+  if (zero_a != nullptr && blockIdx.x == 0 && threadIdx.x == 0) { *zero_a = 0; *zero_b = 0; }
   const int64_t total = B * L, stride = (int64_t)gridDim.x * blockDim.x;
   for (int64_t t = (int64_t)blockIdx.x * blockDim.x + threadIdx.x; t < total; t += stride) {
     const int64_t b = t / L;
@@ -1051,6 +1055,8 @@
   const void* g_first = nullptr;
   void* grad_first = nullptr;
   int32_t* long_rows = nullptr;
+  bool zero_in_build = false;
+  int32_t* split_count = nullptr;
   void* tg = nullptr;
   float* scratch = nullptr;
   RowSink sink = GRAD_SINK;
@@ -1066,16 +1072,17 @@
   bool scal = false;
   const void* fm = j.g_fm;
   if (j.g_fm != nullptr && j.fm_sum != nullptr) {
+    int32_t* zero_a = j.zero_in_build ? j.long_rows : nullptr;
     if (j.g_fm_cols == 1) {
       uint4* gvec = (uint4*)j.tg + j.B * L;
       hipLaunchKernelGGL((build_tg1_kernel<T>), dim3(stream_grid(j.B * L, 256, 4096)), dim3(256), 0, s,
-                         (const T*)j.g_fm, j.fm_sum, (uint4*)j.tg, gvec, j.B, L);
+                         (const T*)j.g_fm, j.fm_sum, (uint4*)j.tg, gvec, j.B, L, zero_a, j.split_count);
       fs = FmSrc{(const uint4*)j.tg, gvec, L, 1};
       fs.g1 = j.g_fm;
       scal = j.g_first == nullptr;
     } else {
       hipLaunchKernelGGL((build_tg_kernel<T>), dim3(stream_grid(j.B * L, 256, 4096)), dim3(256), 0, s,
-                         (const uint4*)j.g_fm, j.fm_sum, (uint4*)j.tg, j.B, L);
+                         (const uint4*)j.g_fm, j.fm_sum, (uint4*)j.tg, j.B, L, zero_a, j.split_count);
       fs = FmSrc{(const uint4*)j.tg, (const uint4*)j.tg + L, 2 * L, 2 * L};
     }
     fm = j.tg;
@@ -1339,8 +1346,9 @@
   j.long_rows = (int32_t*)workspace;
   j.tg = (char*)workspace + long_row_queue_bytes(BN);
   j.scratch = (float*)((char*)j.tg + align_up((size_t)j.B * 2 * j.E * dtype_size(dtype), 256));
-  hipLaunchKernelGGL(zero_two_i32_kernel, dim3(1), dim3(64), 0, j.s, j.long_rows,
-                     j.long_rows + 1 + (BN / LONG_ROW_ELEM + 2));
+  j.split_count = j.long_rows + 1 + (BN / LONG_ROW_ELEM + 2);
+  j.zero_in_build = lg >= 0 && j.g_fm != nullptr && j.fm_sum != nullptr;
+  if (!j.zero_in_build) hipLaunchKernelGGL(zero_two_i32_kernel, dim3(1), dim3(64), 0, j.s, j.long_rows, j.split_count);
   return dtype == TRS_F32 ? scatter_launch<float>(j, lg) : scatter_launch<bf16_t>(j, lg);
 }
 
diff --git a/torecsys_amd/functional.py b/torecsys_amd/functional.py
--- a/torecsys_amd/functional.py
+++ b/torecsys_amd/functional.py
@@ -3018,18 +3018,20 @@
 
 def fused_mlp_backward_raw(gy2: torch.Tensor, widths: Sequence[int], Ws: Sequence[torch.Tensor],
                            masks: Sequence[torch.Tensor], mask_in: Optional[torch.Tensor] = None, *, family: int,
-                           h_last: Optional[torch.Tensor] = None, live: int = 0):
+                           h_last: Optional[torch.Tensor] = None, live: int = 0, parts: bool = False):
     if family not in (MLP_FAMILY_TILE, MLP_FAMILY_ROW_OWNER, MLP_FAMILY_MIXED):
         raise ValueError("fused_mlp_backward_raw: family must be the value the forward returned with these masks")
     L = len(Ws)
     rows, dev = gy2.shape[0], gy2.device
     gz = [torch.empty(rows, _pad32(widths[l + 1]), dtype=torch.bfloat16, device=dev) for l in range(L - 1)]
-    gb = [torch.empty(_pad32(widths[l + 1]), dtype=torch.float32, device=dev) for l in range(L)]
     gx = torch.empty(rows, widths[0], dtype=torch.bfloat16, device=dev)
-    gb_in = torch.empty(_pad32(widths[0]), dtype=torch.float32, device=dev) if mask_in is not None else None
     wl = _i32_array(widths)
     ws_bytes = size_query("trs_mlp_fused_workspace_bytes", L, wl)
     ws = torch.empty(ws_bytes, dtype=torch.uint8, device=dev)
+    if parts:
+        return _fused_mlp_backward_parts(gy2, widths, Ws, masks, mask_in, family, h_last, live, gz, gx, wl, ws)
+    gb = [torch.empty(_pad32(widths[l + 1]), dtype=torch.float32, device=dev) for l in range(L)]
+    gb_in = torch.empty(_pad32(widths[0]), dtype=torch.float32, device=dev) if mask_in is not None else None
     if h_last is not None:
         if not (gy2.is_contiguous() and h_last.is_contiguous() and h_last.shape[0] == rows):
             raise ValueError("fused_mlp_backward_raw: gy2 / h_last must be contiguous over the same rows")
@@ -3043,6 +3045,59 @@
     call("trs_mlp_fused_bwd_data", ptr(gy2), rows, L, wl, _ptr_array(Ws), _ptr_array(masks), _ptr_array(gz),
          _ptr_array(gb), ptr(gx), ptr(mask_in), ptr(gb_in), _abi.TRS_BF16, int(family), ptr(ws), ws_bytes, stream_ptr())
     return gx, gz, gb, gb_in
+
+
+def _fused_mlp_backward_parts(gy2, widths, Ws, masks, mask_in, family, h_last, live, gz, gx, wl, ws):
+    L, rows, dev = len(Ws), gy2.shape[0], gy2.device
+    part, part_bytes = None, 0
+    if h_last is not None:
+        if not (gy2.is_contiguous() and h_last.is_contiguous() and h_last.shape[0] == rows):
+            raise ValueError("fused_mlp_backward_raw: gy2 / h_last must be contiguous over the same rows")
+        part_bytes = mlp_bwd_wlast_bytes(widths, max(rows, 1), family, live)
+        part = torch.empty(max(part_bytes, 16), dtype=torch.uint8, device=dev)
+    n = L + 4
+    where, stride, nparts = (ctypes.c_void_p * n)(), (ctypes.c_int32 * n)(), ctypes.c_int32(0)
+    call("trs_mlp_fused_bwd_data_parts", ptr(gy2), gy2.shape[1], rows, L, wl, _ptr_array(Ws), _ptr_array(masks),
+         _ptr_array(gz), ptr(gx), ptr(mask_in), ptr(h_last), h_last.shape[1] if h_last is not None else 0, int(live),
+         ptr(part), part_bytes, where, stride, ctypes.byref(nparts),
+         _abi.TRS_BF16, int(family), ptr(ws), ws.numel(), stream_ptr())
+    P = int(nparts.value)
+
+    def view(base, k, shape, strides):
+        f32 = base.view(torch.float32)
+        off = (int(where[k] or 0) - base.data_ptr()) // 4
+        last = off + sum((s - 1) * st for s, st in zip(shape, strides))
+        if not (where[k] and 0 <= off and last < f32.numel()):
+            raise RuntimeError("fused_mlp_backward_raw: a partial set lies outside its buffer")
+        return torch.as_strided(f32, shape, strides, off)
+
+    gb = [view(ws, l, (P, _pad32(widths[l + 1])), (int(stride[l]), 1)) for l in range(L)]
+    gb_in = view(ws, L, (P, _pad32(widths[0])), (int(stride[L]), 1)) if mask_in is not None else None
+    out = [gx, gz, gb, gb_in]
+    if h_last is not None:
+        Kh = _pad32(widths[L - 1])
+        out.append(view(part, L + 1, (P, live, Kh), (int(stride[L + 1]), Kh, 1)))
+    return tuple(out)
+
+
+def colsum_parts_reduce(sets: Sequence[torch.Tensor]) -> List[torch.Tensor]:
+    outs = [torch.empty(t.shape[1], dtype=torch.float32, device=t.device) for t in sets]
+    if len({t.shape[0] for t in sets}) != 1 or any(t.dim() != 2 or t.stride(1) != 1 for t in sets):
+        raise ValueError("colsum_parts_reduce: sets of one launch share their partial count")
+    call("trs_colsum_parts_reduce", len(sets), _ptr_array(sets), _i32_array([t.stride(0) for t in sets]),
+         _i32_array([t.shape[1] for t in sets]), int(sets[0].shape[0]), _ptr_array(outs), stream_ptr())
+    return outs
+
+
+def _plain_sum(t):
+    return colsum_parts_reduce([t])[0] if t is not None and t.dim() == 2 else t
+
+
+def _parts_arrays(srcs):
+    if not any(t is not None and t.dim() == 2 for t in srcs):
+        return None
+    return (_i32_array([t.shape[0] if t is not None and t.dim() == 2 else 0 for t in srcs]),
+            _i32_array([t.stride(0) if t is not None and t.dim() == 2 else 0 for t in srcs]))
 
 
 class _FusedMLP(Function):
@@ -3165,6 +3220,16 @@
                       _i32_array([j[1].shape[1] for j in jobs]), int(jobs[0][0].shape[0]))
 
 
+def wgrad_deep_splits_for(rows: int, dims) -> int:
+    if not WGRAD_ROWS or not 2 <= len(dims) <= 4 or rows < DEEP_WGRAD_MIN_ROWS:
+        return 0
+    M_x, N_g = [(d[0] + 207) // 208 * 208 for d in dims], [(d[2] + 15) // 16 * 16 for d in dims]
+    if any(m > d[1] or n > d[3] for m, n, d in zip(M_x, N_g, dims)):
+        return 0
+    return size_query("trs_wgrad_wide_many_splits", len(dims), _i32_array(M_x), _i32_array([d[1] for d in dims]),
+                      _i32_array(N_g), _i32_array([d[3] for d in dims]), int(rows))
+
+
 def _wgrad_deep(jobs, S, casts):
     dev, rows = jobs[0][0].device, int(jobs[0][0].shape[0])
     parts = [torch.empty(S, j[2], j[3], dtype=torch.float32, device=dev) for j in jobs]
@@ -3174,11 +3239,14 @@
     gws = [torch.empty(j[4], j[5], dtype=torch.bfloat16, device=dev) for j in jobs]
     gbs = [torch.empty(j[4], dtype=torch.bfloat16, device=dev) if j[6] is not None else None for j in jobs]
     n = len(casts)
-    call("trs_wgrad_finish_t_many", len(jobs) + n, _ptr_array(parts + [None] * n), S,
+    srcs = [j[6] for j in jobs] + [c[1] for c in casts]
+    sets = _parts_arrays(srcs)
+    call("trs_wgrad_finish_t_many" if sets is None else "trs_wgrad_finish_t_many_parts", len(jobs) + n,
+         _ptr_array(parts + [None] * n), S,
          _i32_array([j[2] for j in jobs] + [0] * n), _i32_array([j[3] for j in jobs] + [0] * n),
          _i32_array([j[4] for j in jobs] + [0] * n), _i32_array([j[5] for j in jobs] + [c[0] for c in casts]),
-         _abi.TRS_BF16, _ptr_array(gws + [None] * n), _ptr_array([j[6] for j in jobs] + [c[1] for c in casts]),
-         _ptr_array(gbs + [c[2] for c in casts]), stream_ptr())
+         _abi.TRS_BF16, _ptr_array(gws + [None] * n), _ptr_array(srcs),
+         _ptr_array(gbs + [c[2] for c in casts]), *(sets or ()), stream_ptr())
     return list(zip(gws, gbs))
 
 
@@ -3195,14 +3263,18 @@
         _, _, out_f, in_f, dt, gb_f32, _, need_b = layers[-1]
         gw = torch.empty(out_f, in_f, dtype=dt, device=gw_last.device)
         gbias = torch.empty(out_f, dtype=dt, device=gw_last.device) if need_b else None
-        casts = [(in_f, gw_last[r], gw[r]) for r in range(out_f)] + ([(out_f, gb_f32, gbias)] if need_b else [])
+        casts = [(in_f, gw_last[r] if gw_last.dim() == 2 else gw_last[:, r], gw[r]) for r in range(out_f)] + \
+                ([(out_f, gb_f32, gbias)] if need_b else [])
         out[-1] = (gw, gbias)
 
     def finish(parts, S, R, Cc, orows, ocols, gws, gbfs, gbs, dtype_code, extra):
         n = len(extra)
-        call("trs_wgrad_finish_many", len(parts) + n, _ptr_array(parts + [None] * n), S, _i32_array(R + [0] * n),
+        srcs = gbfs + [c[1] for c in extra]
+        sets = _parts_arrays(srcs)
+        call("trs_wgrad_finish_many" if sets is None else "trs_wgrad_finish_many_parts", len(parts) + n,
+             _ptr_array(parts + [None] * n), S, _i32_array(R + [0] * n),
              _i32_array(Cc + [0] * n), _i32_array(orows + [0] * n), _i32_array(ocols + [c[0] for c in extra]), dtype_code,
-             _ptr_array(gws + [None] * n), _ptr_array(gbfs + [c[1] for c in extra]), _ptr_array(gbs + [c[2] for c in extra]),
+             _ptr_array(gws + [None] * n), _ptr_array(srcs), _ptr_array(gbs + [c[2] for c in extra]), *(sets or ()),
              stream_ptr())
 
     first_out = None
@@ -3234,13 +3306,13 @@
         for n, k in enumerate(batch):
             gb = gbs[n]
             if gb is None and layers[k][7]:
-                gb = layers[k][5][:layers[k][2]].to(dtype)
+                gb = _plain_sum(layers[k][5])[:layers[k][2]].to(dtype)
             out[k] = (gws[n], gb)
     if casts:
         finish([], 1, [], [], [], [], [], [], [], value_dtype_code(casts[0][2]), casts)
     for k, t in enumerate(layers):
         if out[k] is None:
-            out[k] = _tail_layer_grads(*t)
+            out[k] = _tail_layer_grads(*t[:5], _plain_sum(t[5]) if t[7] else None, *t[6:])
     return out if first is None else out + [first_out]
 
 
diff --git a/torecsys_amd/layers.py b/torecsys_amd/layers.py
--- a/torecsys_amd/layers.py
+++ b/torecsys_amd/layers.py
@@ -723,7 +723,7 @@
     if need_x and F_.rows_gemm_supported(g2, W, out_f, xin.shape[1]) and W.shape[1] == xin.shape[1]:
         gx = F_.rows_gemm(g2, W, out_f, xin.shape[1])
     elif need_x:
-        gx = g2 @ W
+        gx = g2 @ W if g2.shape[1] == W.shape[0] else g2[:, :out_f] @ W[:out_f]
     return gx, gw_out, gb_out
 
 
@@ -746,8 +746,10 @@
         else:
             y, hidden, masks, mask_in, fam = F_.fused_mlp_forward_raw(h1, Ws, bs, input_mask=True)
         out_f = tail[4 * (L - 1)].shape[0]
+        if w_narrow is not None:
+            Ws = [w_narrow] + Ws[1:]
         ctx.save_for_backward(cur, W1, h1, mask_in, *Ws, *hidden, *masks)
-        ctx.meta = (L, [h1.shape[1]] + [w.shape[0] for w in Ws], [tuple(tail[4 * l].shape) for l in range(L)],
+        ctx.meta = (L, [Ws[0].shape[1]] + [w.shape[0] for w in Ws], [tuple(tail[4 * l].shape) for l in range(L)],
                     [tail[4 * l].dtype for l in range(L)], tuple(w1.shape), w1.dtype, tuple(x.shape), fam)
         y = y[:, :out_f] if out_f != y.shape[1] else y
         return y.reshape(*x.shape[:-1], out_f)
@@ -763,8 +765,20 @@
         needs = ctx.needs_input_grad
         gy = gy.reshape(h1.shape[0], -1)
         live, gw_last = wshapes[L - 1][0], None
-        if (needs[6 + 4 * (L - 1)] and gy.dtype == torch.bfloat16 and gy.shape[1] == live
-                and F_.mlp_bwd_wlast_bytes(widths, h1.shape[0], fam, live) > 0):
+        rows = h1.shape[0]
+        carried = (needs[6 + 4 * (L - 1)] and gy.dtype == torch.bfloat16 and gy.shape[1] == live
+                   and F_.mlp_bwd_wlast_bytes(widths, rows, fam, live) > 0)
+        tail_w = [l for l in range(L - 1) if needs[6 + 4 * l]]
+        merged = (carried and needs[2] and tail_w and w1dt == torch.bfloat16 and all(d == torch.bfloat16 for d in wdt)
+                  and fam in (F_.MLP_FAMILY_TILE, F_.MLP_FAMILY_MIXED) and cur.dtype == h1.dtype == torch.bfloat16
+                  and F_.wgrad_deep_splits_for(rows, [(w1shape[1], cur.shape[1], w1shape[0], widths[0])] + [
+                      (wshapes[l][1], (h1 if l == 0 else hidden[l - 1]).shape[1], wshapes[l][0], F_._pad32(widths[l + 1]))
+                      for l in tail_w]) > 0)
+        if merged:
+            gy2 = gy.contiguous()
+            g1, gz, gb, gb1, gw_last = F_.fused_mlp_backward_raw(gy2, widths, Ws, masks, mask_in, family=fam,
+                                                                 h_last=hidden[L - 2], live=live, parts=True)
+        elif carried:
             gy2 = gy.contiguous()
             g1, gz, gb, gb1, gw_last = F_.fused_mlp_backward_raw(gy2, widths, Ws, masks, mask_in, family=fam,
                                                                  h_last=hidden[L - 2], live=live)
@@ -777,6 +791,8 @@
                                      first=(g1, cur, w1shape[0], w1shape[1], w1dt, gb1, needs[2], needs[3]))
         for gw, gbias in tail:
             grads += [gw, gbias, None, None]
+        if done is None or (needs[3] and done[1] is None):
+            gb1 = F_._plain_sum(gb1)
         gx, gw1, gbias1 = _dense_layer_grads(g1, gb1, cur, W1, w1shape[0], w1shape[1], w1dt, needs[0], needs[2], needs[3],
                                              done)
         return (gx.reshape(xshape) if needs[0] else None, None, gw1, gbias1, None, None, *grads)
```

Result: faster. 68.06 million samples/s, median of 6 (+1.6%).
